# fdrmrc/Polydeal

Hardware: AMD Instinct MI355X
Metric: assembled DoF/s (SIP Poisson, p=3, 3D) (higher is better)
Workload: dtype f64

## Files before the change

polydeal_amd/csrc/pdh_capi.cpp:

```cpp
#include "pdh_basis.h"
#include "pdh_combos.h"
#include "pdh_ctx.h"
#include "pdh_kernels.h"
#include "pdh_moment_tables.h"

#include <hip/hip_runtime.h>

#include <algorithm>
#include <chrono>
#include <cmath>
#include <cstdio>
#include <cstdlib>
#include <cstring>
#include <memory>
#include <string>
#include <vector>

static pdh_resolve_fn g_resolve[PDH_N_GROUPS] = {pdh_resolve_g0, pdh_resolve_g1, pdh_resolve_g2, pdh_resolve_g3,
                                                 pdh_resolve_g4, pdh_resolve_g5, pdh_resolve_g6, pdh_resolve_g7};

template <int NT, int LB>
static constexpr int sched_instr(bool sym)
{
  int c = 0;
// ... 80 lines not shown
    (void)hipHostFree(ctx->pinned);
  for (auto &ev : ctx->events)
    if (ev)
      (void)hipEventDestroy(ev);
  (void)hipStreamDestroy(ctx->own_stream);
  if (ctx->stream2)
    (void)hipStreamDestroy(ctx->stream2);
  if (ctx->ev_fork)
    (void)hipEventDestroy(ctx->ev_fork);
  if (ctx->ev_join)
    (void)hipEventDestroy(ctx->ev_join);
  delete ctx;
}

extern "C" int pdh_terms_merge_stats(pdh_ctx *ctx, int64_t *out4)
{
  if (!ctx || !out4)
    return fail(ctx, PDH_EINVAL, "ctx and out4 are required");
  if (!ctx->prob.resident)
    return fail(ctx, PDH_ESTATE, "pdh_terms_merge_stats called before pdh_set_problem");
  for (int i = 0; i < 4; ++i)
    out4[i] = ctx->prob.row_kernel == RowKernel::terms ? ctx->prob.terms_merge[i] : 0;
  return PDH_OK;
}

struct GaussRule01
{
  double x[PDH_MAX_N1D] = {0}, w[PDH_MAX_N1D] = {0};
  explicit GaussRule01(int n)
  {
    std::vector<long double> gx, gw;
    pdh::gauss_legendre01(n, gx, gw);
    for (int i = 0; i < n; ++i)
      x[i] = (double)gx[i], w[i] = (double)gw[i];
  }
};

static int pack_faces_on_device(pdh_ctx *ctx, const pdh_problem *p, const Packed &K, PdhDev &D)
{
  const int dim = p->dim;
  const int64_t nap = K.n_ap, nqf = K.nqf_src, nruns = (int64_t)K.pk_at.size();
  double *out[5] = {nullptr, nullptr, nullptr, nullptr, nullptr};
  const size_t out_n[5] = {(size_t)dim * nap, (size_t)dim * nap, (size_t)nap, (size_t)nap, (size_t)nap};
  for (int k = 0; k < 5; ++k)
    PDH_TRY(device_buffer(ctx, out_n[k], &out[k], "packed face points"));
  D.ap_x = out[0], D.ap_n = out[1], D.ap_wself = out[2], D.ap_wcross = out[3], D.ap_sig = out[4];
  if (nruns == 0 || nap == 0)
    return PDH_OK;
  Staging st(ctx);
  const double *d_x = nullptr, *d_n = nullptr, *d_w = nullptr, *d_wo = nullptr;
  if (K.cart)
    {
      const pdh_cartesian_points *cp = K.cart;
      const int64_t nsf = nqf / ((int64_t)cp->nqf * cp->nqf);
      const double *d_box = nullptr;
      const int32_t *d_cell = nullptr, *d_face = nullptr;
      double *x = nullptr, *n = nullptr, *w = nullptr;
      PDH_TRY(st.upload(cp->cell_box, (size_t)cp->n_cells * 6, &d_box, "cell boxes"));
      PDH_TRY(st.upload(cp->fq_cell, (size_t)nsf, &d_cell, "cells of the sub-faces"));
      PDH_TRY(st.upload(cp->fq_face, (size_t)nsf, &d_face, "local faces of the sub-faces"));
      PDH_TRY(st.alloc((size_t)dim * nqf, &x, "face points"));
      PDH_TRY(st.alloc((size_t)dim * nqf, &n, "face normals"));
      PDH_TRY(st.alloc((size_t)nqf, &w, "face weights"));
      const GaussRule01 g(cp->nqf);
      PDH_HIP(ctx, pdh_launch_gen_faces(cp->nqf, g.x, g.w, d_box, d_cell, d_face, nqf, x, n, w, ctx->stream));
      d_x = x, d_n = n, d_w = w;
    }
  else
    {
      PDH_TRY(st.upload(p->fq_x, (size_t)dim * nqf, &d_x, "face points"));
      PDH_TRY(st.upload(p->fq_n, (size_t)dim * nqf, &d_n, "face normals"));
      PDH_TRY(st.upload(p->fq_w, (size_t)nqf, &d_w, "face weights"));
      if (p->fq_w_out)
        PDH_TRY(st.upload(p->fq_w_out, (size_t)nqf, &d_wo, "face weights of side 1"));
    }
  const int64_t *d_at = nullptr, *d_fq = nullptr;
  const int32_t *d_cnt = nullptr, *d_fl = nullptr;
  const double *d_sg = nullptr;
  PDH_TRY(st.upload(K.pk_at.data(), K.pk_at.size(), &d_at, "face runs: packed position"));
  PDH_TRY(st.upload(K.pk_fq.data(), K.pk_fq.size(), &d_fq, "face runs: caller position"));
  PDH_TRY(st.upload(K.pk_cnt.data(), K.pk_cnt.size(), &d_cnt, "face runs: counts"));
  PDH_TRY(st.upload(K.pk_flags.data(), K.pk_flags.size(), &d_fl, "face runs: flags"));
  PDH_TRY(st.upload(K.pk_sig.data(), K.pk_sig.size(), &d_sg, "face runs: sigma"));
  PDH_HIP(ctx, pdh_launch_pack_faces(dim, nqf, d_x, d_n, d_w, d_wo, nruns, d_at, d_fq, d_cnt, d_fl, d_sg, nap, out[0], out[1], out[2],
                                     out[3], out[4], ctx->stream));
  PDH_HIP(ctx, hipStreamSynchronize(ctx->stream));
  return PDH_OK;
}

static int generate_volume_points(pdh_ctx *ctx, const Packed &K, PdhDev &D)
{
  const pdh_cartesian_points *cart = K.cart;
  const int64_t m3 = (int64_t)cart->nq * cart->nq * cart->nq, ngroups = K.n_vq / m3;
  std::vector<int32_t> gcell((size_t)std::max<int64_t>(ngroups, 1));
  for (int sl = 0; sl < K.n_owned; ++sl)
    {
      const int64_t g0 = K.vq_ptr[sl] / m3, g1 = K.vq_ptr[sl + 1] / m3, src = K.vq_src[sl] / m3;
      for (int64_t g = g0; g < g1; ++g)
        gcell[(size_t)g] = cart->vq_cell[src + (g - g0)];
    }
  double *x = nullptr, *w = nullptr;
  PDH_TRY(device_buffer(ctx, (size_t)3 * K.n_vq, &x, "volume points"));
  PDH_TRY(device_buffer(ctx, (size_t)K.n_vq, &w, "volume weights"));
  Staging st(ctx);
  const double *d_box = nullptr;
  const int32_t *d_gcell = nullptr;
  PDH_TRY(st.upload(cart->cell_box, (size_t)cart->n_cells * 6, &d_box, "cell boxes"));
  PDH_TRY(st.upload(gcell.data(), gcell.size(), &d_gcell, "cells of the volume rules"));
  const GaussRule01 g(cart->nq);
  PDH_HIP(ctx, pdh_launch_gen_volume(cart->nq, g.x, g.w, d_box, d_gcell, K.n_vq, x, K.n_vq, w, ctx->stream));
  PDH_HIP(ctx, hipStreamSynchronize(ctx->stream));
  D.vq_x = x, D.vq_w = w;
  return PDH_OK;
}

static int upload_problem(pdh_ctx *ctx, const pdh_problem *p, const Packed &K)
{
  PdhDev &D = ctx->prob.dev;
  std::memset(&D, 0, sizeof(D));
  D.dim = p->dim;
  D.n = K.n;
  D.n1d = K.n1d;
  D.diag_first = p->diag_first ? 1 : 0;
  D.reaction_c = p->reaction_c;
  D.tab = K.tab;
  D.vq_stride = K.vq_stride_h;
  D.ap_stride = K.n_ap;
  const std::vector<double> bbox(p->bbox, p->bbox + (size_t)p->n_agg * 2 * p->dim);
  PDH_UP(bbox, D.bbox);
  PDH_UP(K.midx, D.midx);
  PDH_UP(K.vq_ptr, D.vq_ptr);
  if (K.cart)
    PDH_TRY(generate_volume_points(ctx, K, D));
  else
    {
      PDH_TRY(upload(ctx, K.vqx_h, (size_t)p->dim * K.vq_stride_h, &D.vq_x, "D.vq_x"));
      PDH_TRY(upload(ctx, K.vqw_h, (size_t)K.n_vq, &D.vq_w, "D.vq_w"));
    }
  PDH_UP(K.ap_ptr, D.ap_ptr);
  PDH_TRY(pack_faces_on_device(ctx, p, K, D));
  PDH_UP(K.own_agg, D.own_agg);
  PDH_UP(K.own_row, D.own_row);
  PDH_UP(K.row_base, D.row_base);
  PDH_UP(K.row_len, D.row_len);
  PDH_UP(K.diag_L, D.diag_L);
  PDH_UP(K.it_own, D.it_own);
  PDH_UP(K.it_nbr, D.it_nbr);
  PDH_UP(K.it_pbeg, D.it_pbeg);
  PDH_UP(K.it_pcnt, D.it_pcnt);
  PDH_UP(K.it_pos, D.it_pos);
  PDH_UP(K.it_nbr_slot, D.it_nbr_slot);
  PDH_UP(K.it_pos_t, D.it_pos_t);
  PDH_TRY(upload(ctx, K.blk_ptr, &ctx->prob.d_blk_ptr, "ctx->d_blk_ptr"));
  PDH_TRY(upload(ctx, K.blk_dof, &ctx->prob.d_blk_dof, "ctx->d_blk_dof"));
  if (K.ghost)
    {
      PDH_TRY(upload(ctx, K.r21_src, &ctx->prob.d_r21_src, "ctx->d_r21_src"));
      PDH_TRY(upload(ctx, K.r21_dst, &ctx->prob.d_r21_dst, "ctx->d_r21_dst"));
      PDH_TRY(upload(ctx, K.r21_rlen, &ctx->prob.d_r21_rlen, "ctx->d_r21_rlen"));
      PDH_TRY(upload(ctx, K.r22_ptr, &ctx->prob.d_r22_ptr, "ctx->d_r22_ptr"));
      PDH_TRY(upload(ctx, K.r22_src, &ctx->prob.d_r22_src, "ctx->d_r22_src"));
      PDH_TRY(upload(ctx, K.r22_slot, &ctx->prob.d_r22_slot, "ctx->d_r22_slot"));
    }
  PDH_TRY(device_buffer(ctx, (size_t)(K.n_values + K.n_send), &D.values, "values"));
  PDH_TRY(upload(ctx, K.vq_src, &ctx->prob.d_vq_src, "ctx->d_vq_src"));
  if (p->dim == 3 && K.n1d >= 2 && K.n1d <= 4)
    {
      const std::vector<double> mt = pdh::moment_tables(p->degree, p->basis);
      if ((int)mt.size() != pdhm::moment_table_doubles(K.n1d))
        return fail(ctx, PDH_EDEVICE, "moment tables: the host's and the kernels' sizes differ");
      PDH_TRY(upload(ctx, mt, &ctx->prob.d_mtab, "ctx->d_mtab"));
    }
  return PDH_OK;
}

static void record_problem(pdh_ctx *ctx, const pdh_problem *p, const Packed &K)
{
  ctx->prob.ghost = K.ghost;
  ctx->prob.n_send = K.n_send;
  ctx->prob.n_recv = K.n_recv;
  ctx->prob.send_count = K.send_count;
  ctx->prob.recv_count = K.recv_count;
  ctx->prob.n_r21 = (int)K.r21_src.size();
  ctx->prob.n_r22 = (int)K.r22_slot.size();
  ctx->prob.n_values = K.n_values;
  ctx->prob.n_owned = K.n_owned;
  ctx->prob.n_diag_slots = (int)K.own_agg.size();
  ctx->prob.n_items = (int)K.it_own.size();
  ctx->prob.n_vq = K.n_vq;
  ctx->prob.n_ap = K.n_ap;
  ctx->prob.NT = K.NT;
  ctx->prob.tiled = K.tiled;
  ctx->prob.basis = p->basis;
  ctx->prob.n_vq_caller = p->vq_ptr[p->n_agg];
  ctx->prob.n_fq_caller = p->n_faces ? p->fq_ptr[p->n_faces] : 0;
  ctx->prob.cart_fq_face.clear();
  ctx->prob.cart_nqf = 0;
  if (K.cart && K.cart->nqf > 0)
    {
      ctx->prob.cart_nqf = K.cart->nqf;
      ctx->prob.cart_fq_face.assign(K.cart->fq_face, K.cart->fq_face + ctx->prob.n_fq_caller / ((int64_t)K.cart->nqf * K.cart->nqf));
    }
  ctx->prob.face_runs.clear();
  ctx->prob.face_runs.reserve(K.run_ap.size());
  for (size_t r = 0; r < K.run_ap.size(); ++r)
    ctx->prob.face_runs.push_back({K.run_ap[r], K.run_fq[r], K.run_cnt[r], K.run_bdry[r], K.run_slot[r]});
  ctx->prob.n_rows_owned = (int64_t)K.n_owned * K.n;
  ctx->prob.n_rows_total = p->n_rows;
  ctx->prob.max_row_len = K.max_row_len;
  ctx->prob.h_blk_ptr = K.blk_ptr;
  ctx->prob.h_blk_dof = K.blk_dof;
  ctx->prob.h_slot_dof.resize((size_t)K.n_owned);
  for (int s = 0; s < K.n_owned; ++s)
    ctx->prob.h_slot_dof[(size_t)s] = p->dof_offset[K.own_agg[(size_t)s]];
  ctx->prob.n_agg_total = p->n_agg;
  const int64_t i_sym = sched_instr_rt(K.NT, K.LB, true), i_full = sched_instr_rt(K.NT, K.LB, false);
  const int ch_d = (K.NT >= 3) ? 64 : 32, ch_o = 32;
  auto ksteps = [](int64_t npts, int ch) {
    int64_t s = (npts / ch) * (ch / 4);
    const int64_t rem = npts % ch;
    return s + (rem + 3) / 4;
  };
  int64_t kv = 0, kf = 0, ko = 0;
  for (size_t sl = 0; sl < K.own_agg.size(); ++sl)
    {
      kv += ksteps(K.vq_ptr[sl + 1] - K.vq_ptr[sl], ch_d);
      kf += ksteps(K.ap_ptr[sl + 1] - K.ap_ptr[sl], ch_d);
    }
  for (size_t it = 0; it < K.it_pcnt.size(); ++it)
    ko += ksteps(K.it_pcnt[it], ch_o);
  ctx->prob.mfma_diag = kv * (p->dim + (p->reaction_c != 0.0 ? 1 : 0)) * i_sym + kf * 2 * i_sym;
  ctx->prob.mfma_offdiag = ko * 2 * i_full;
  if (K.tiled)
    {
      const int64_t nt = (K.n + 63) / 64, i64 = sched_instr_rt(4, 4, true);
      ctx->prob.mfma_diag = (kv * (p->dim + (p->reaction_c != 0.0 ? 1 : 0)) + kf * 2) * (64 * (nt * (nt - 1) / 2) + i64 * nt);
      ctx->prob.mfma_offdiag = ko * 2 * 64 * nt * nt;
    }
}

static int upload_rows_state(pdh_ctx *ctx, const Packed &K, const KernelPlan &plan, int cus)
{
  const RowsHost &RH = plan.rows;
  PdhRows &R = ctx->prob.rows;
  PDH_UP(RH.fr_ptr, R.fr_ptr);
  PDH_UP(RH.fr_pbeg, R.fr_pbeg);
  PDH_UP(RH.fr_pcnt, R.fr_pcnt);
  PDH_UP(RH.fr_nbr, R.fr_nbr);
  PDH_UP(RH.fr_axis, R.fr_axis);
  PDH_UP(RH.fr_blk, R.fr_blk);
  PDH_UP(RH.fr_flags, R.fr_flags);
  PDH_UP(RH.fr_coord, R.fr_coord);
  PDH_UP(RH.fr_sigma, R.fr_sigma);
  PDH_UP(RH.fr_nsign, R.fr_nsign);
  PDH_UP(RH.meta, R.meta);
  PDH_TRY(device_buffer(ctx, 16, &R.sched, "row kernel: work counter"));
  PDH_HIP(ctx, hipMemset(R.sched, 0, 16 * sizeof(unsigned int)));
  const size_t n_stamps = (size_t)std::max(K.n_owned, 1) * 16;
  PDH_TRY(device_buffer(ctx, n_stamps, &R.stamps, "row kernel: stamps"));
  PDH_HIP(ctx, hipMemset(R.stamps, 0, n_stamps * sizeof(long long)));
  if (RH.multi)
    {
      const int waves = cus * 8;
      const size_t stride = std::max<size_t>((size_t)RH.maxf * 64, (size_t)RH.maxs * 32 + 64);
      PDH_TRY(device_buffer(ctx, (size_t)waves * stride, &R.m2c_scratch, "row kernel: MULTI scratch"));
      R.scratch_waves = waves;
      R.scratch_stride = (int64_t)stride;
    }
  R.tensor_only = plan.tensor_only ? 1 : 0;
  R.multi = RH.multi ? 1 : 0;
  R.maxe = RH.maxe;
  R.maxf = RH.maxf;
  R.vq_tensor_n = plan.vq_n;
  R.fq_tensor_n = RH.fq_tensor_n;
  return PDH_OK;
}

static int upload_terms_state(pdh_ctx *ctx, const Packed &K, const KernelPlan &plan)
{
  const TermsHost &TH = plan.terms;
  PdhTerms &T = ctx->prob.terms;
  PDH_UP(TH.meta, T.meta);
  PDH_UP(TH.sf_pt, T.sf_pt);
  PDH_UP(TH.sf_info, T.sf_info);
  PDH_UP(TH.sf_ivl, T.sf_ivl);
  PDH_UP(TH.cell_ivl, T.cell_ivl);
  T.maxruns = TH.maxruns, T.maxsf = TH.maxsf, T.maxsi = TH.maxsi, T.maxcell = TH.maxcell;
  T.vq_tensor_n = plan.vq_n, T.fq_tensor_n = plan.rows.fq_tensor_n;
  T.lds_bytes = TH.lds_bytes;
  T.split = TH.split;
  T.task_pts = TH.task_pts;
  T.tpm = TH.task_pts > 4 ? 8 : 4;
  T.tstride = pdht::terms_task_doubles(T.maxsf, T.maxcell, T.tpm);
  const size_t n_tdata = (size_t)std::max(K.n_owned, 1) * T.tstride;
  double *tdata = nullptr;
  PDH_TRY(device_buffer(ctx, n_tdata, &tdata, "term kernel: records of 1-D rules"));
  PDH_HIP(ctx, hipMemsetAsync(tdata, 0, n_tdata * sizeof(double), ctx->stream));
  T.tdata = tdata;
  PDH_HIP(ctx, pdh_launch_terms_gather(&ctx->prob.dev, &T, tdata, K.n_owned, ctx->stream));
  PDH_HIP(ctx, hipStreamSynchronize(ctx->stream));
  const size_t n_stamps = (size_t)std::max(K.n_owned, 1) * 16;
  PDH_TRY(device_buffer(ctx, n_stamps, &T.stamps, "term kernel: stamps"));
  PDH_HIP(ctx, hipMemset(T.stamps, 0, n_stamps * sizeof(long long)));
  ctx->prob.terms_merge[0] = TH.n_cells_in, ctx->prob.terms_merge[1] = TH.n_cells_out;
  ctx->prob.terms_merge[2] = TH.n_sf_in, ctx->prob.terms_merge[3] = TH.n_sf_out;
  return PDH_OK;
}

static void resolve_launches(pdh_ctx *ctx, const Packed &K, const PlanSwitches &sw, int cus)
{
  pdh_ctx::Problem &pr = ctx->prob;
  const PdhDev &D = pr.dev;
  const bool reaction = D.reaction_c != 0.0;
  if (K.tiled)
    pdh_resolve_tiled(D.dim, D.n1d, D.n, reaction, pr.n_diag_slots, pr.n_items, pr.direct);
  else
    g_resolve[combo_group(D.dim, D.n1d, K.NT, K.LB)](D.dim, D.n1d, K.NT, K.LB, reaction, pr.n_diag_slots, pr.n_items, pr.direct);
  if (pr.d_mtab)
    pdh_resolve_moment(D.n1d, D.n, pr.n_diag_slots, pr.n_items, pr.moment);
  if (pr.row_kernel == RowKernel::rows)
    pr.row = pdh_resolve_rows(&D, &pr.rows, pr.n_owned, cus, sw.rows_waves_per_cu, sw.rows_lds_pad, sw.rows_verbose, &pr.row_zero_sched);
  else if (pr.row_kernel == RowKernel::terms)
    pr.row = pdh_resolve_terms(&D, &pr.terms, pr.n_owned, sw.terms_wg_waves);
}

static int set_problem_impl(pdh_ctx *ctx, const pdh_problem *p, int32_t row_begin, int32_t row_end, const pdh_cartesian_points *cart);

extern "C" int pdh_set_problem_local(pdh_ctx *ctx, const pdh_problem *p, int32_t row_begin, int32_t row_end)
{
  return set_problem_impl(ctx, p, row_begin, row_end, nullptr);
}

extern "C" int pdh_set_problem_cartesian(pdh_ctx *ctx, const pdh_problem *p, const pdh_cartesian_points *points, int32_t row_begin,
                                         int32_t row_end)
{
  if (!points)
    return fail(ctx, PDH_EINVAL, "points is NULL");
  return set_problem_impl(ctx, p, row_begin, row_end, points);
}

static int set_problem_impl(pdh_ctx *ctx, const pdh_problem *p, int32_t row_begin, int32_t row_end, const pdh_cartesian_points *cart)
{
  PDH_TRY(need_ctx(ctx));
  if (cart && ctx->exchange_mode == PDH_EXCHANGE_GHOST)
    return fail(ctx, PDH_EUNSUPPORTED, "the cartesian description runs owner-computes-rows only (no ghost-block exchange)");
  PDH_HIP(ctx, hipSetDevice(ctx->device));
  PDH_HIP(ctx, hipStreamSynchronize(ctx->stream));
  free_problem(ctx);
  ++ctx->values_gen;
  ++ctx->problem_epoch;
  struct FreeUnlessDone
  {
    pdh_ctx *ctx;
    bool done = false;
    ~FreeUnlessDone()
    {
      if (!done)
        free_problem(ctx);
    }
  } guard{ctx};
  const PlanSwitches sw = read_plan_switches();
  auto t_last = std::chrono::steady_clock::now();
  auto lap = [&](const char *what) {
    if (!sw.trace)
      return;
    const auto now = std::chrono::steady_clock::now();
    fprintf(stderr, "[pdh_set_problem] %-32s %7.1f ms\n", what, std::chrono::duration<double, std::milli>(now - t_last).count());
    t_last = now;
  };
  lap("wait for the stream, free the old problem");

  std::unique_ptr<Packed> K_owner(new Packed);
  Packed &K = *K_owner;
  PDH_TRY(pack_problem(ctx->err, p, row_begin, row_end, K, ctx->exchange_mode, cart));
  lap("validate + repack (host)");
  auto plan = std::make_unique<KernelPlan>(plan_kernels(p, K, sw));
  lap("row kernel plan (host)");
  if (cart && plan->kernel != RowKernel::terms)
    return fail(ctx, PDH_EUNSUPPORTED, "cartesian description: the term kernels do not apply (a polytope's tables exceed their LDS budget, "
                                       "or the element has none): describe the problem with its points (pdh_set_problem)");
  PDH_TRY(upload_problem(ctx, p, K));
  record_problem(ctx, p, K);
  lap("upload: state of every kernel");
  int cus = 256;
  (void)hipDeviceGetAttribute(&cus, hipDeviceAttributeMultiprocessorCount, ctx->device);
  if (plan->kernel == RowKernel::rows)
    {
      PDH_TRY(upload_rows_state(ctx, K, *plan, cus));
      lap("upload: pdh_rows.h state");
    }
  else if (plan->kernel == RowKernel::terms)
    {
      PDH_TRY(upload_terms_state(ctx, K, *plan));
      lap("upload: term kernel state");
    }
  ctx->prob.row_kernel = plan->kernel;
  ctx->prob.why_terms = plan->why_terms;
  resolve_launches(ctx, K, sw, cus);
  ctx->prob.resident = true;
  ctx->ev_used = 0;
  guard.done = true;
  K_owner.reset();
  plan.reset();
  lap("release host staging");
  return PDH_OK;
}

extern "C" int pdh_set_algorithm(pdh_ctx *ctx, int algorithm)
{
  PDH_TRY(need_ctx(ctx));
  if (algorithm != PDH_ALG_AUTO && algorithm != PDH_ALG_DIRECT && algorithm != PDH_ALG_MOMENT && algorithm != PDH_ALG_ROWS)
    return fail(ctx, PDH_EINVAL, "algorithm must be PDH_ALG_AUTO, PDH_ALG_DIRECT, PDH_ALG_MOMENT or PDH_ALG_ROWS");
  ctx->algorithm = algorithm;
  return PDH_OK;
}

extern "C" int pdh_algorithm_in_use(pdh_ctx *ctx)
{
  if (!resident(ctx))
    return fail(ctx, PDH_ESTATE, "no problem resident");
  if (ctx->use_rows())
    return PDH_ALG_ROWS;
  const bool d = ctx->use_moment(0), o = ctx->use_moment(1);
  return d && o ? PDH_ALG_MOMENT : (d || o ? PDH_ALG_MIXED : PDH_ALG_DIRECT);
}

extern "C" int pdh_rows_kernel_in_use(pdh_ctx *ctx)
{
  if (!resident(ctx))
    return fail(ctx, PDH_ESTATE, "no problem resident");
  if (!ctx->use_rows())
    return PDH_ROWS_NONE;
  if (ctx->prob.row_kernel == RowKernel::terms)
    return PDH_ROWS_TERMS;
  if (ctx->prob.rows.multi)
    return PDH_ROWS_MULTI;
  return ctx->prob.dev.n == 64 ? PDH_ROWS_PIECES : PDH_ROWS_STREAMED;
}

extern "C" int pdh_set_problem(pdh_ctx *ctx, const pdh_problem *p)
{
  if (!p)
    return fail(ctx, PDH_EINVAL, "problem is NULL");
  return pdh_set_problem_local(ctx, p, 0, p->n_rows);
}

static int take_events(pdh_ctx *ctx, hipEvent_t (&e)[4])
{
  for (hipEvent_t &x : e)
    x = ctx->next_event();
  if (!e[0] || !e[1] || !e[2] || !e[3])
    return fail(ctx, PDH_EDEVICE, "hipEventCreate failed");
  return PDH_OK;
}

extern "C" int pdh_assemble_device(pdh_ctx *ctx)
{
  PDH_TRY(need_problem(ctx, "pdh_assemble_device"));
  ++ctx->values_gen;
  PDH_HIP(ctx, hipSetDevice(ctx->device));
  pdh_ctx::Problem &pr = ctx->prob;
  if (ctx->algorithm == PDH_ALG_MOMENT && !ctx->prob.d_mtab)
    return fail(ctx, PDH_EUNSUPPORTED, "the moment form exists for 3-D bases of degree 1..3 only");
  if (ctx->algorithm == PDH_ALG_ROWS && ctx->prob.row_kernel == RowKernel::none)
    return fail(ctx, PDH_EUNSUPPORTED, "the row kernel does not apply to the resident problem (3-D FE_DGQ / FE_AggloDGP of degree 1 .. 3 on polytopes whose faces are unions of axis-aligned planes, no exchange variant; pdh_check_rows says why)");
  pr.has_values = true;
  pr.galerkin_values = false;
  if (ctx->use_rows())
    {
      hipEvent_t ev[4] = {nullptr, nullptr, nullptr, nullptr};
      if (ctx->profiling)
        {
          PDH_TRY(take_events(ctx, ev));
          PDH_HIP(ctx, hipEventRecord(ev[0], ctx->stream));
        }
      if (pr.row_kernel == RowKernel::terms)
        PDH_HIP(ctx, pdh_launch_terms(&pr.row, &pr.dev, &pr.terms, pr.n_owned, ctx->stream));
      else
        PDH_HIP(ctx, pdh_launch_rows(&pr.row, pr.row_zero_sched, &pr.dev, &pr.rows, pr.d_mtab, pr.n_owned, ctx->stream));
      if (ctx->profiling)
        {
          PDH_HIP(ctx, hipEventRecord(ev[1], ctx->stream));
          PDH_HIP(ctx, hipEventRecord(ev[2], ctx->stream));
          PDH_HIP(ctx, hipEventRecord(ev[3], ctx->stream));
        }
      return PDH_OK;
    }
  hipEvent_t ev[4] = {nullptr, nullptr, nullptr, nullptr};
  if (ctx->profiling)
    PDH_TRY(take_events(ctx, ev));
  hipEvent_t e0 = ev[0], e1 = ev[1], f0 = ev[2], f1 = ev[3];
  const bool ov = ctx->overlapped();
  hipStream_t sd = ctx->stream, so = ov ? ctx->stream2 : ctx->stream;
  const bool graphable = !ctx->profiling && !ov && ctx->prob.n_values < pdh_ctx::small_values;
  if (graphable && ctx->prob.graph_state == 1 && (ctx->prob.graph_alg != ctx->algorithm || ctx->prob.graph_stream != ctx->stream))
    ctx->prob.drop_graph();
  if (graphable && ctx->prob.graph_state == 1)
    {
      PDH_HIP(ctx, hipGraphLaunch(ctx->prob.graph_exec, ctx->stream));
      return PDH_OK;
    }
  bool capturing = false;
  if (graphable && ctx->prob.graph_state == 0)
    {
      if (hipStreamBeginCapture(ctx->stream, hipStreamCaptureModeThreadLocal) == hipSuccess)
        capturing = true;
      else
        {
          (void)hipGetLastError();
          ctx->prob.graph_state = -1;
        }
    }
  auto end_capture = [&](bool ok) {
    if (!capturing)
      return;
    hipGraph_t g = nullptr;
    hipError_t e = hipStreamEndCapture(ctx->stream, &g);
    if (ok && e == hipSuccess && g && hipGraphInstantiate(&ctx->prob.graph_exec, g, nullptr, nullptr, 0) == hipSuccess)
      {
        ctx->prob.graph_state = 1;
        ctx->prob.graph_alg = ctx->algorithm;
        ctx->prob.graph_stream = ctx->stream;
      }
    else
      {
        (void)hipGetLastError();
        ctx->prob.graph_exec = nullptr;
        ctx->prob.graph_state = -1;
      }
    if (g)
      (void)hipGraphDestroy(g);
  };
  auto launch_blocks = [&](int k, int count, hipStream_t s) {
    if (ctx->use_moment(k))
      return pdh_launch_moment(&pr.moment[k], &pr.dev, pr.d_mtab, count, s);
    if (!pr.tiled)
      return pdh_launch_direct(&pr.direct[k], &pr.dev, count, s);
    const hipError_t e = pdh_launch_tiled(&pr.direct[k], &pr.dev, count, s);
    return k == 0 && e == hipSuccess ? pdh_launch_tiled(&pr.direct[2], &pr.dev, count, s) : e;
  };
  if (ov)
    {
      PDH_HIP(ctx, hipEventRecord(ctx->ev_fork, ctx->stream));
      PDH_HIP(ctx, hipStreamWaitEvent(ctx->stream2, ctx->ev_fork, 0));
    }
  if (ctx->profiling)
    PDH_HIP(ctx, hipEventRecord(e0, sd));
  {
    const hipError_t le = launch_blocks(0, pr.n_diag_slots, sd);
    if (le != hipSuccess)
      {
        end_capture(false);
        return fail(ctx, PDH_EDEVICE, std::string("diagonal-block kernel: ") + hipGetErrorString(le));
      }
  }
  if (ctx->profiling)
    PDH_HIP(ctx, hipEventRecord(e1, sd));
  if (ctx->profiling)
    PDH_HIP(ctx, hipEventRecord(f0, so));
  {
    const hipError_t le = launch_blocks(1, pr.n_items, so);
    if (le != hipSuccess)
      {
        end_capture(false);
        return fail(ctx, PDH_EDEVICE, std::string("coupling-block kernel: ") + hipGetErrorString(le));
      }
  }
  if (ctx->profiling)
    PDH_HIP(ctx, hipEventRecord(f1, so));
  if (ov)
    {
      PDH_HIP(ctx, hipEventRecord(ctx->ev_join, ctx->stream2));
      PDH_HIP(ctx, hipStreamWaitEvent(ctx->stream, ctx->ev_join, 0));
    }
  if (capturing)
    {
      end_capture(true);
      if (ctx->prob.graph_state == 1)
        PDH_HIP(ctx, hipGraphLaunch(ctx->prob.graph_exec, ctx->stream));
      else
        return pdh_assemble_device(ctx);
    }
  return PDH_OK;
}

extern "C" int pdh_set_exchange_mode(pdh_ctx *ctx, int mode)
{
  PDH_TRY(need_ctx(ctx));
  if (mode != PDH_EXCHANGE_NONE && mode != PDH_EXCHANGE_GHOST)
    return fail(ctx, PDH_EINVAL, "mode must be PDH_EXCHANGE_NONE or PDH_EXCHANGE_GHOST");
  ctx->exchange_mode = mode;
  return PDH_OK;
}

extern "C" int pdh_exchange_layout(pdh_ctx *ctx, int n_ranks, int64_t *send_count, int64_t *recv_count)
{
  if (!resident(ctx))
    return fail(ctx, PDH_ESTATE, "no problem resident");
  if (!ctx->prob.ghost)
    return fail(ctx, PDH_ESTATE, "the resident problem was not set in PDH_EXCHANGE_GHOST mode");
  if (n_ranks < (int)ctx->prob.send_count.size() || !send_count || !recv_count)
    return fail(ctx, PDH_EINVAL, "n_ranks is smaller than the number of ranks in agg_rank, or an output is NULL");
  for (int r = 0; r < n_ranks; ++r)
    {
      send_count[r] = r < (int)ctx->prob.send_count.size() ? ctx->prob.send_count[r] : 0;
      recv_count[r] = r < (int)ctx->prob.recv_count.size() ? ctx->prob.recv_count[r] : 0;
    }
  return PDH_OK;
}

extern "C" int pdh_exchange_get_send(pdh_ctx *ctx, double *d_send)
{
  if (!resident(ctx) || !ctx->prob.ghost)
    return fail(ctx, PDH_ESTATE, "no problem resident in PDH_EXCHANGE_GHOST mode");
  if (ctx->prob.n_send == 0)
    return PDH_OK;
  if (!d_send)
    return fail(ctx, PDH_EINVAL, "d_send is NULL");
  PDH_HIP(ctx, hipSetDevice(ctx->device));
  PDH_HIP(ctx, hipMemcpyAsync(d_send, ctx->prob.dev.values + ctx->prob.n_values, ctx->prob.n_send * sizeof(double), hipMemcpyDeviceToDevice,
                              ctx->stream));
  return PDH_OK;
}

extern "C" int pdh_exchange_apply(pdh_ctx *ctx, const double *d_recv)
{
  if (!resident(ctx) || !ctx->prob.ghost)
    return fail(ctx, PDH_ESTATE, "no problem resident in PDH_EXCHANGE_GHOST mode");
  ++ctx->values_gen;
  if (ctx->prob.n_recv == 0)
    return PDH_OK;
  if (!d_recv)
    return fail(ctx, PDH_EINVAL, "d_recv is NULL");
  PDH_HIP(ctx, hipSetDevice(ctx->device));
  PDH_HIP(ctx, pdh_launch_ghost_apply(&ctx->prob.dev, d_recv, ctx->prob.n_r21, ctx->prob.d_r21_src, ctx->prob.d_r21_dst, ctx->prob.d_r21_rlen, ctx->prob.n_r22,
                                      ctx->prob.d_r22_ptr, ctx->prob.d_r22_src, ctx->prob.d_r22_slot, ctx->stream));
  return PDH_OK;
}

extern "C" int pdh_set_stream(pdh_ctx *ctx, void *stream)
{
  PDH_TRY(need_ctx(ctx));
  PDH_HIP(ctx, hipSetDevice(ctx->device));
  PDH_HIP(ctx, hipStreamSynchronize(ctx->stream));
  ctx->stream = stream ? (hipStream_t)stream : ctx->own_stream;
  return PDH_OK;
}

extern "C" int pdh_debug_rows_stamps(pdh_ctx *ctx, long long *out)
{
  const long long *src = !ctx || !ctx->prob.resident ? nullptr
                         : ctx->prob.row_kernel == RowKernel::terms ? ctx->prob.terms.stamps
                         : ctx->prob.row_kernel == RowKernel::rows ? ctx->prob.rows.stamps
                                                                : nullptr;
  if (!src || !out)
    return fail(ctx, PDH_ESTATE, "no row-kernel problem resident");
  PDH_HIP(ctx, hipSetDevice(ctx->device));
  PDH_HIP(ctx, hipStreamSynchronize(ctx->stream));
  PDH_HIP(ctx, hipMemcpy(out, src, (size_t)ctx->prob.n_owned * 16 * sizeof(long long), hipMemcpyDeviceToHost));
  return PDH_OK;
}

extern "C" int pdh_set_overlap(pdh_ctx *ctx, int enabled)
{
  PDH_TRY(need_ctx(ctx));
  ctx->overlap = enabled != 0;
  return PDH_OK;
}

extern "C" int pdh_synchronize(pdh_ctx *ctx)
{
  PDH_TRY(need_ctx(ctx));
  PDH_HIP(ctx, hipSetDevice(ctx->device));
  PDH_HIP(ctx, hipStreamSynchronize(ctx->stream));
  return PDH_OK;
}

extern "C" void *pdh_stream(pdh_ctx *ctx) { return ctx ? (void *)ctx->stream : nullptr; }

extern "C" int pdh_assemble(pdh_ctx *ctx, double *values)
{
  if (!values)
    return fail(ctx, PDH_EINVAL, "values is NULL");
  int rc = pdh_assemble_device(ctx);
  if (rc != PDH_OK)
    return rc;
  PDH_HIP(ctx, hipMemcpyAsync(values, ctx->prob.dev.values, ctx->prob.n_values * sizeof(double), hipMemcpyDeviceToHost, ctx->stream));
  PDH_HIP(ctx, hipStreamSynchronize(ctx->stream));
  return PDH_OK;
}

extern "C" int pdh_copy_values(pdh_ctx *ctx, double *values)
{
  if (!resident(ctx))
    return fail(ctx, PDH_ESTATE, "no problem resident");
  if (!values)
    return fail(ctx, PDH_EINVAL, "values is NULL");
  PDH_HIP(ctx, hipSetDevice(ctx->device));
  PDH_HIP(ctx, hipMemcpyAsync(values, ctx->prob.dev.values, ctx->prob.n_values * sizeof(double), hipMemcpyDeviceToHost, ctx->stream));
  PDH_HIP(ctx, hipStreamSynchronize(ctx->stream));
  return PDH_OK;
}

extern "C" int pdh_values_checksum(pdh_ctx *ctx, double *out4)
{
  if (!resident(ctx))
    return fail(ctx, PDH_ESTATE, "no problem resident");
  if (!out4)
    return fail(ctx, PDH_EINVAL, "out4 is NULL");
  PDH_HIP(ctx, hipSetDevice(ctx->device));
  double *d = ctx->checksum.get<double>(4);
  if (!d)
    return fail(ctx, PDH_EDEVICE, "pdh_values_checksum: out of device memory");
  hipError_t e = pdh_launch_checksum(ctx->prob.dev.values, ctx->prob.n_values, d, ctx->stream);
  if (e == hipSuccess)
    e = hipMemcpyAsync(out4, d, 4 * sizeof(double), hipMemcpyDeviceToHost, ctx->stream);
  if (e == hipSuccess)
    e = hipStreamSynchronize(ctx->stream);
  if (e != hipSuccess)
    return fail(ctx, PDH_EDEVICE, std::string("pdh_values_checksum: ") + hipGetErrorString(e));
  return PDH_OK;
}

extern "C" int pdh_assemble_sip_local(pdh_ctx *ctx, const pdh_problem *p, int32_t row_begin, int32_t row_end, double *values)
{
  int rc = pdh_set_problem_local(ctx, p, row_begin, row_end);
  if (rc != PDH_OK)
    return rc;
  return pdh_assemble(ctx, values);
}

extern "C" int pdh_assemble_sip(pdh_ctx *ctx, const pdh_problem *p, double *values)
{
  if (!p)
    return fail(ctx, PDH_EINVAL, "problem is NULL");
  return pdh_assemble_sip_local(ctx, p, 0, p->n_rows, values);
}
extern "C" int pdh_device_values(pdh_ctx *ctx, double **device_ptr, int64_t *n_values)
{
  if (!resident(ctx))
    return fail(ctx, PDH_ESTATE, "no problem resident");
  if (device_ptr)
    *device_ptr = ctx->prob.dev.values;
  if (n_values)
    *n_values = ctx->prob.n_values;
  return PDH_OK;
}

extern "C" int pdh_set_profiling(pdh_ctx *ctx, int enabled)
{
  PDH_TRY(need_ctx(ctx));
  PDH_HIP(ctx, hipSetDevice(ctx->device));
  PDH_HIP(ctx, hipStreamSynchronize(ctx->stream));
  ctx->profiling = enabled != 0;
  ctx->ev_used = 0;
  return PDH_OK;
}

extern "C" int pdh_kernel_times_ms(pdh_ctx *ctx, float *ms, int *n_launches)
{
  if (!ctx || !ms)
    return fail(ctx, PDH_EINVAL, "ctx or ms is NULL");
  const size_t nl = ctx->ev_used / 4;
  if (nl == 0)
    return fail(ctx, PDH_ESTATE, "no profiled launch recorded (pdh_set_profiling(1) then pdh_assemble_device)");
  PDH_HIP(ctx, hipSetDevice(ctx->device));
  PDH_HIP(ctx, hipStreamSynchronize(ctx->stream));
  double sum[PDH_N_KERNELS] = {0.0, 0.0};
  for (size_t l = 0; l < nl; ++l)
    for (int k = 0; k < PDH_N_KERNELS; ++k)
      {
        float t = 0.f;
        PDH_HIP(ctx, hipEventElapsedTime(&t, ctx->events[4 * l + 2 * k], ctx->events[4 * l + 2 * k + 1]));
        sum[k] += t;
      }
  for (int k = 0; k < PDH_N_KERNELS; ++k)
    ms[k] = (float)(sum[k] / (double)nl);
  if (n_launches)
    *n_launches = (int)nl;
  return PDH_OK;
}

extern "C" int pdh_kernel_work(pdh_ctx *ctx, int64_t *mfma_instr)
{
  if (!resident(ctx) || !mfma_instr)
    return fail(ctx, PDH_ESTATE, "no problem resident");
  mfma_instr[0] = (ctx->use_moment(0) || ctx->use_rows()) ? 0 : ctx->prob.mfma_diag;
  mfma_instr[1] = (ctx->use_moment(1) || ctx->use_rows()) ? 0 : ctx->prob.mfma_offdiag;
  return PDH_OK;
}

extern "C" int pdh_problem_stats(pdh_ctx *ctx, int64_t *stats)
{
  if (!resident(ctx) || !stats)
    return fail(ctx, PDH_ESTATE, "no problem resident");
  stats[0] = ctx->prob.n_owned;
  stats[1] = ctx->prob.n_items;
  stats[2] = ctx->prob.n_vq;
  stats[3] = ctx->prob.n_ap;
  stats[4] = ctx->prob.n_values;
  stats[5] = ctx->prob.dev.n;
  stats[6] = (int64_t)pdh::lds_bytes_diag(ctx->prob.dev.dim, ctx->prob.dev.n1d, ctx->prob.NT);
  stats[7] = (int64_t)pdh::lds_bytes_offdiag(ctx->prob.dev.dim, ctx->prob.dev.n1d, ctx->prob.NT);
  return PDH_OK;
}
```

polydeal_amd/csrc/pdh_exchange.hip:

```cpp
#include "pdh_kernels.h"
#include "pdh_launch.h"

__global__ void __launch_bounds__(PDH_WAVE) k_ghost_apply(const PdhDev P, const double *__restrict__ recv, const int n_r21,
                                                          const int64_t *__restrict__ r21_src, const int64_t *__restrict__ r21_dst,
                                                          const int32_t *__restrict__ r21_rlen, const int n_r22,
                                                          const int64_t *__restrict__ r22_ptr, const int64_t *__restrict__ r22_src,
                                                          const int32_t *__restrict__ r22_slot)
{
  const int lane = threadIdx.x, item = blockIdx.x, n = P.n;
  if (lane >= n)
    return;
  if (item < n_r21)
    {
      const double *src = recv + r21_src[item] + lane;
      double *dst = P.values + r21_dst[item] + lane;
      const int64_t rlen = r21_rlen[item];
      for (int R = 0; R < n; ++R)
        dst[R * rlen] = src[(int64_t)R * n];
    }
  else if (item < n_r21 + n_r22)
    {
      const int k = item - n_r21, slot = r22_slot[k];
      const int64_t rlen = P.row_len[slot];
      const int dest = (P.diag_first && lane == 0) ? 0 : P.diag_L[slot] + lane;
      double *dst = P.values + P.row_base[slot] + dest;
      const int64_t sb = r22_ptr[k], se = r22_ptr[k + 1];
      for (int R = 0; R < n; ++R)
        {
          double acc = dst[R * rlen];
          for (int64_t s = sb; s < se; ++s)
            acc += recv[r22_src[s] + (int64_t)R * n + lane];
          dst[R * rlen] = acc;
        }
    }
}

extern "C" hipError_t pdh_launch_ghost_apply(const PdhDev *P, const double *recv, int n_r21, const int64_t *r21_src,
                                             const int64_t *r21_dst, const int32_t *r21_rlen, int n_r22, const int64_t *r22_ptr,
                                             const int64_t *r22_src, const int32_t *r22_slot, hipStream_t stream)
{
  const int count = n_r21 + n_r22;
  if (count <= 0)
    return hipSuccess;
  hipLaunchKernelGGL(k_ghost_apply, dim3((unsigned)count), dim3(PDH_WAVE), 0, stream, *P, recv, n_r21, r21_src, r21_dst, r21_rlen,
                     n_r22, r22_ptr, r22_src, r22_slot);
  return hipGetLastError();
}

__global__ void __launch_bounds__(256) k_checksum(const double *__restrict__ v, const int64_t n, double *__restrict__ out)
{
  double s = 0.0, sa = 0.0, mx = 0.0, bad = 0.0;
  for (int64_t i = (int64_t)blockIdx.x * blockDim.x + threadIdx.x; i < n; i += (int64_t)gridDim.x * blockDim.x)
    {
      const double x = v[i];
      if (isfinite(x))
        {
          s += x;
          sa += fabs(x);
          mx = fmax(mx, fabs(x));
        }
      else
        bad += 1.0;
    }
  for (int o = 32; o > 0; o >>= 1)
    {
      s += __shfl_down(s, o);
      sa += __shfl_down(sa, o);
      bad += __shfl_down(bad, o);
      mx = fmax(mx, __shfl_down(mx, o));
    }
  if ((threadIdx.x & 63) == 0)
    {
      atomicAdd(out + 0, s);
      atomicAdd(out + 1, sa);
      atomicAdd(out + 3, bad);
      atomicMax(reinterpret_cast<unsigned long long *>(out + 2), (unsigned long long)__double_as_longlong(mx));
    }
}

extern "C" hipError_t pdh_launch_checksum(const double *values, int64_t n, double *d_out4, hipStream_t stream)
{
  hipError_t e = hipMemsetAsync(d_out4, 0, 4 * sizeof(double), stream);
  if (e != hipSuccess || n <= 0)
    return e;
  hipLaunchKernelGGL(k_checksum, dim3(2048), dim3(256), 0, stream, values, n, d_out4);
  return hipGetLastError();
}

__global__ void __launch_bounds__(256) k_pack_faces(const int dim, const int64_t nqf, const double *__restrict__ fq_x,
                                                    const double *__restrict__ fq_n, const double *__restrict__ fq_w,
                                                    const double *__restrict__ fq_w_out, const int64_t n_runs,
                                                    const int64_t *__restrict__ pk_at, const int64_t *__restrict__ pk_fq,
                                                    const int32_t *__restrict__ pk_cnt, const int32_t *__restrict__ pk_flags,
                                                    const double *__restrict__ pk_sig, const int64_t nap, double *__restrict__ ap_x,
                                                    double *__restrict__ ap_n, double *__restrict__ ap_wself,
                                                    double *__restrict__ ap_wcross, double *__restrict__ ap_sig)
{
  const int lane = threadIdx.x & (PDH_WAVE - 1);
  const int64_t r = (int64_t)blockIdx.x * (blockDim.x / PDH_WAVE) + (threadIdx.x / PDH_WAVE);
  if (r >= n_runs)
    return;
  const int64_t at = pk_at[r], fq = pk_fq[r];
  const int cnt = pk_cnt[r], fl = pk_flags[r];
  const bool side0 = (fl & 1) != 0, bdry = (fl & 2) != 0;
  const double sig = pk_sig[r], sgn = side0 ? 1.0 : -1.0;
  for (int t = lane; t < cnt; t += PDH_WAVE)
    {
      const int64_t q = fq + t, a = at + t;
      const double w_in = fq_w[q], w_out = fq_w_out ? fq_w_out[q] : w_in;
      ap_wself[a] = bdry ? 2.0 * w_in : (side0 ? w_in : w_out);
      ap_wcross[a] = bdry ? 0.0 : w_out;
      ap_sig[a] = sig;
      for (int c = 0; c < dim; ++c)
        {
          ap_x[c * nap + a] = fq_x[c * nqf + q];
          ap_n[c * nap + a] = sgn * fq_n[c * nqf + q];
        }
    }
}

extern "C" hipError_t pdh_launch_pack_faces(int dim, int64_t nqf, const double *fq_x, const double *fq_n, const double *fq_w,
                                            const double *fq_w_out, int64_t n_runs, const int64_t *pk_at, const int64_t *pk_fq,
                                            const int32_t *pk_cnt, const int32_t *pk_flags, const double *pk_sig, int64_t nap,
                                            double *ap_x, double *ap_n, double *ap_wself, double *ap_wcross, double *ap_sig,
                                            hipStream_t stream)
{
  if (n_runs <= 0)
    return hipSuccess;
  const int per_block = 256 / PDH_WAVE;
  const int64_t blocks = (n_runs + per_block - 1) / per_block;
  hipLaunchKernelGGL(k_pack_faces, dim3((unsigned)blocks), dim3(256), 0, stream, dim, nqf, fq_x, fq_n, fq_w, fq_w_out, n_runs, pk_at,
                     pk_fq, pk_cnt, pk_flags, pk_sig, nap, ap_x, ap_n, ap_wself, ap_wcross, ap_sig);
  return hipGetLastError();
}
```

polydeal_amd/csrc/pdh_launch.h:

```cpp
#pragma once
#include <hip/hip_runtime.h>
#include <stdint.h>

#include <type_traits>

#include "pdh_dev.h"
#include "pdh_rows_tables.h"
#include "pdh_solve.h"
#include "pdh_terms_tables.h"

struct PdhTransferArgs;
struct PdhGalerkinArgs;

struct PdhLaunch
{
  const void *kernel;
  unsigned grid, block;
  size_t lds;
};

typedef void (*PdhDirectKernel)(PdhDev, int);
typedef void (*PdhTiledKernel)(PdhDev, int, int);
typedef void (*PdhMomentKernel)(PdhDev, const double *, int);
typedef void (*PdhRowsKernel)(PdhDev, PdhRows, const double *, int);
typedef void (*PdhTermsKernel)(PdhDev, PdhTerms, int);

template <class... A>
inline PdhLaunch pdh_record(void (*kernel)(A...), long long grid, unsigned block, size_t lds)
{
  return grid > 0x7fffffffLL ? PdhLaunch{} : PdhLaunch{(const void *)kernel, (unsigned)(grid > 0 ? grid : 0), block, lds};
}
template <class... A>
inline hipError_t pdh_launch_as(void (*)(A...), const PdhLaunch &L, hipStream_t stream, A... a)
{
  if (!L.kernel)
    return hipErrorInvalidValue;
  if (!L.grid)
    return hipSuccess;
  void *args[] = {&a...};
  (void)hipLaunchKernel(L.kernel, dim3(L.grid), dim3(L.block), args, L.lds, stream);
  return hipGetLastError();
}
template <class F>
inline void pdh_for_bools(F &&f)
{
  f();
}
template <class F, class... B>
inline void pdh_for_bools(F &&f, bool b, B... rest)
{
  if (b)
    pdh_for_bools([&](auto... c) { f(std::true_type{}, c...); }, rest...);
  else
    pdh_for_bools([&](auto... c) { f(std::false_type{}, c...); }, rest...);
}

extern "C" {
typedef void (*pdh_resolve_fn)(int dim, int n1d, int nt, int lb, bool reaction, int n_own, int n_items, PdhLaunch *L);
#define PDH_DECL(g) void pdh_resolve_g##g(int, int, int, int, bool, int, int, PdhLaunch *);
PDH_DECL(0) PDH_DECL(1) PDH_DECL(2) PDH_DECL(3) PDH_DECL(4) PDH_DECL(5) PDH_DECL(6) PDH_DECL(7)
#undef PDH_DECL
hipError_t pdh_launch_direct(const PdhLaunch *L, const PdhDev *P, int count, hipStream_t stream);

hipError_t pdh_launch_rhs(int dim, int n1d, const PdhDev *P, int count, const double *f_vol, const double *g_face, double *rhs,
                          const int64_t *vq_src, const int64_t *ap_src, const int64_t *bd_rng, hipStream_t stream);

hipError_t pdh_launch_eval(int dim, int n1d, int grad, const PdhDev *P, int count, const double *coef, const int64_t *pt_ptr,
                           const double *pts, int64_t pts_stride, double *out_u, double *out_g, int by_agg, hipStream_t stream);
hipError_t pdh_launch_shape(int dim, int n1d, const PdhDev *P, int n_boxes, const int64_t *pt_ptr, const double *pts,
                            int64_t pts_stride, double *out, hipStream_t stream);
hipError_t pdh_launch_eval_err(int dim, int n1d, const PdhDev *P, int count, const double *coef, const int64_t *pt_ptr,
                               const double *pts, int64_t pts_stride, const double *w, const double *exact_u, const double *exact_g,
                               double *err, hipStream_t stream);

void pdh_resolve_moment(int n1d, int n, int n_own, int n_items, PdhLaunch *L);
hipError_t pdh_launch_moment(const PdhLaunch *L, const PdhDev *P, const double *mtab, int count, hipStream_t stream);
PdhLaunch pdh_resolve_rows(const PdhDev *P, const PdhRows *R, int count, int cus, int waves_per_cu, size_t lds_pad, bool verbose,
                           bool *zero_sched);
hipError_t pdh_launch_rows(const PdhLaunch *L, bool zero_sched, const PdhDev *P, const PdhRows *R, const double *mtab, int count,
                           hipStream_t stream);

PdhLaunch pdh_resolve_terms(const PdhDev *P, const PdhTerms *T, int count, int wg_waves);
hipError_t pdh_launch_terms(const PdhLaunch *L, const PdhDev *P, const PdhTerms *T, int count, hipStream_t stream);
hipError_t pdh_launch_terms_gather(const PdhDev *P, const PdhTerms *T, double *out, int count, hipStream_t stream);

hipError_t pdh_launch_mf_tables(const PdhDev *P, const PdhTerms *T, double *tables, int count, hipStream_t stream);
hipError_t pdh_launch_mf_vmult(const PdhSolveArgs *A, int n1d, const PdhTerms *T, const double *tables, const double *x, double *y,
                               double *part, hipStream_t stream);

void pdh_resolve_tiled(int dim, int n1d, int n, bool reaction, int n_own, int n_items, PdhLaunch *L);
hipError_t pdh_launch_tiled(const PdhLaunch *L, const PdhDev *P, int count, hipStream_t stream);

hipError_t pdh_launch_gen_volume(int nq, const double *nodes, const double *weights, const double *d_box, const int32_t *d_gcell,
                                 int64_t n_points, double *vq_x, int64_t stride, double *vq_w, hipStream_t stream);
hipError_t pdh_launch_gen_faces(int nqf, const double *nodes, const double *weights, const double *d_box, const int32_t *d_cell,
                                const int32_t *d_face, int64_t n_points, double *fq_x, double *fq_n, double *fq_w, hipStream_t stream);

hipError_t pdh_launch_pack_faces(int dim, int64_t nqf, const double *fq_x, const double *fq_n, const double *fq_w,
                                 const double *fq_w_out, int64_t n_runs, const int64_t *pk_at, const int64_t *pk_fq,
                                 const int32_t *pk_cnt, const int32_t *pk_flags, const double *pk_sig, int64_t nap, double *ap_x,
                                 double *ap_n, double *ap_wself, double *ap_wcross, double *ap_sig, hipStream_t stream);
hipError_t pdh_launch_ghost_apply(const PdhDev *P, const double *recv, int n_r21, const int64_t *r21_src, const int64_t *r21_dst,
                                  const int32_t *r21_rlen, int n_r22, const int64_t *r22_ptr, const int64_t *r22_src,
                                  const int32_t *r22_slot, hipStream_t stream);
hipError_t pdh_launch_checksum(const double *values, int64_t n, double *d_out4, hipStream_t stream);

hipError_t pdh_launch_vmult(const PdhSolveArgs *A, const double *x, double *y, double *part, hipStream_t stream);
hipError_t pdh_launch_block_inverse(const PdhSolveArgs *A, double *dinv, int32_t *flag, hipStream_t stream);
hipError_t pdh_launch_diag_inverse(const PdhSolveArgs *A, double *dinv, int32_t *flag, hipStream_t stream);
hipError_t pdh_launch_cg_update(const PdhSolveArgs *A, int mode, int kind, const double *dinv, const double *b, const double *q,
                                const double *p, double *x, double *r, double *z, const double *scal, double *part, hipStream_t stream);
hipError_t pdh_launch_cheb_update(const PdhSolveArgs *A, int first, int kind, const double *dinv, const double *b, const double *q,
                                  double *d, double *r, double *x, double c1, double c2, int zero_start, const double *rcg, double *part,
                                  hipStream_t stream);
hipError_t pdh_launch_cg_direction(int64_t n_rows, int init, const double *z, double *p, const double *scal, hipStream_t stream);
hipError_t pdh_launch_cg_finalise(const double *part, int n_owned, int stage, double *scal, hipStream_t stream);

hipError_t pdh_launch_dense_gather(const PdhSolveArgs *A, double *D, int ld, int n_rows, hipStream_t stream);
hipError_t pdh_launch_dense_cholesky(double *U, int ld, int n_rows, double *dg, double *piv, int32_t *flag, hipStream_t stream);
hipError_t pdh_launch_dense_inverse(const double *U, const double *dg, int ld, int n_rows, double *Wd, double *G, hipStream_t stream);
hipError_t pdh_launch_dense_symv(const PdhSolveArgs *A, const double *G, int ld, int n_rows, const double *r, double *z,
                                 const double *rcg, double *part, hipStream_t stream);

hipError_t pdh_launch_prolongate(int dim, int n1d, int add, const PdhTransferArgs *A, const double *coarse, double *fine, hipStream_t stream);
hipError_t pdh_launch_restrict(int dim, int n1d, int add, const PdhTransferArgs *A, const double *fine, double *coarse, hipStream_t stream);
hipError_t pdh_launch_residual_sub(int64_t n_rows, const double *b, double *r, hipStream_t stream);

hipError_t pdh_launch_galerkin(int dim, int n1d, const PdhGalerkinArgs *A, hipStream_t stream);
}
```

polydeal_amd/csrc/pdh_plan.cpp:

```cpp
#include "pdh_plan_internal.h"

#include "pdh_basis.h"
#include "pdh_combos.h"
#include "pdh_rows_tables.h"
#include "pdh_terms_tables.h"

#include <chrono>
#include <cstdio>

static thread_local std::string g_err_noctx;
std::string &pdh_noctx_error() { return g_err_noctx; }

int combo_group(int dim, int n1d, int nt, int lb)
{
#define PDH_X(G, D, N, T, L)                                                                       \
  if (dim == D && n1d == N && nt == T && lb == L)                                                  \
    return G;
  PDH_COMBOS(PDH_X)
#undef PDH_X
  return -1;
}


namespace
// ... 1091 lines not shown
  static thread_local std::vector<TermsSfGeom> gs;
  gs.resize((size_t)ns);
  for (int g = 0; g < ns; ++g)
    {
      S.sf_geom(t, g, gs[(size_t)g]);
      gs[(size_t)g].fj = RH.fast_j[3 * t + gs[(size_t)g].c] == 1 ? 1 : 0;
    }
  auto single = [&](int g) {
    TermsMerged::Sf f{};
    f.pb = K.run_ap[t] + g * gsz;
    f.c = gs[(size_t)g].c, f.pos = gs[(size_t)g].pos, f.fj = gs[(size_t)g].fj, f.ni = f.nj = 1;
    out.push_back(f);
  };
  if (mf <= 1 || ns <= 1)
    {
      for (int g = 0; g < ns; ++g)
        single(g);
      return;
    }
  static thread_local std::vector<char> used, ftaken;
  static thread_local std::vector<int> mem, ii, jj, fgrid;
  static thread_local std::vector<double> ki, kj;
  used.assign((size_t)ns, 0);
  for (int g0 = 0; g0 < ns; ++g0)
    {
      if (used[(size_t)g0])
        continue;
      const TermsSfGeom r0 = gs[(size_t)g0];
      mem.clear();
      for (int g = g0; g < ns; ++g)
        if (!used[(size_t)g] && gs[(size_t)g].c == r0.c && gs[(size_t)g].pos == r0.pos && gs[(size_t)g].fj == r0.fj &&
            std::fabs(gs[(size_t)g].z - r0.z) <= 1e-9 * S.hbox[r0.c])
          {
            mem.push_back(g);
            used[(size_t)g] = 1;
          }
      const int c = r0.c, ti = c == 0 ? 1 : 0, tj = c == 2 ? 1 : 2;
      int nd[3] = {0, 0, 1};
      bool ok = mem.size() > 1;
      if (ok)
        {
          ki.resize(mem.size()), kj.resize(mem.size());
          for (size_t m = 0; m < mem.size(); ++m)
            ki[m] = gs[(size_t)mem[m]].xi, kj[m] = gs[(size_t)mem[m]].xj;
          nd[0] = cluster_1d(ki, 1e-9 * S.hbox[ti], ii), nd[1] = cluster_1d(kj, 1e-9 * S.hbox[tj], jj);
          ok = (int64_t)nd[0] * nd[1] <= 4096;
        }
      if (ok)
        {
          fgrid.assign((size_t)nd[0] * nd[1], -1);
          for (size_t m = 0; m < mem.size() && ok; ++m)
            {
              int &gg = fgrid[(size_t)(ii[m] + nd[0] * jj[m])];
              ok = gg < 0;
              gg = (int)m;
            }
        }
      if (!ok)
        {
          for (int g : mem)
            single(g);
          continue;
        }
      auto atm = [&](int i, int j, int = 0) { return fgrid[(size_t)(i + nd[0] * j)]; };
      auto at = [&](int i, int j) { return mem[(size_t)atm(i, j)]; };
      const int mx[3] = {mf, mf, 1};
      ftaken.assign(mem.size(), 0);
      cover_grid(
        nd, mx, ftaken, atm,
        [&](int m, const int *o) {
          return S.sf_fits(t, mem[(size_t)m], at(ii[(size_t)m], o[1]), at(o[0], jj[(size_t)m]), at(o[0], o[1]), ti, tj, r0.fj);
        },
        [&](const int *o, const int *best) {
          TermsMerged::Sf f;
          const int go = at(o[0], o[1]);
          f.pb = K.run_ap[t] + go * gsz;
          f.c = c, f.pos = r0.pos, f.fj = r0.fj;
          f.ni = best[0], f.nj = best[1];
          for (int q = 0; q < TERMS_MI; ++q)
            {
              f.ivl[0][q] = q < best[0] ? (int32_t)((at(o[0] + q, o[1]) - go) * gsz) : 0;
              f.ivl[1][q] = q < best[1] ? (int32_t)((at(o[0], o[1] + q) - go) * gsz) : 0;
            }
          out.push_back(f);
        });
    }
}

template <class Src>
void merge_terms_of_slot(const Src &S, const RowsHost &RH, const std::vector<size_t> &order, bool enabled, TermsMerged &M)
{
  const Packed &K = S.K;
  const int tn = S.tn, fn = S.fn;
  const int ncell = (int)((K.vq_ptr[S.sl + 1] - K.vq_ptr[S.sl]) / S.m3);
  const int mc = tn >= 1 && tn <= 4 ? std::min(TERMS_MI, 8 / tn) : 1;
  if (!(enabled && mc > 1 && ncell > 1 && merge_cells(S, ncell, mc, M.cells)))
    {
      M.cells.resize((size_t)ncell);
      for (int u = 0; u < ncell; ++u)
        for (int d = 0; d < 3; ++d)
          for (int i = 0; i < TERMS_MI; ++i)
            M.cells[(size_t)u].ivl[d][i] = i == 0 ? u : -1;
    }
  const int mf = enabled && fn >= 1 && fn <= 4 ? std::min(TERMS_MI, 8 / fn) : 1;
  M.run_off.assign(order.size() + 1, 0);
  size_t tot = 0;
  for (size_t t : order)
    tot += (size_t)(K.run_cnt[t] / S.gsz);
  M.sfs.reserve(tot);
  M.n_in = ncell + (int64_t)tot;
  for (size_t e = 0; e < order.size(); ++e)
    {
      merge_sub_faces(S, order[e], RH, mf, M.sfs);
      M.run_off[e + 1] = (int)M.sfs.size();
      M.nsf += (int)M.run_size(e);
      if (K.run_nbr[order[e]] >= 0)
        M.nsi += (int)M.run_size(e);
    }
  for (const auto &f : M.sfs)
    M.ivl_f = std::max(M.ivl_f, std::max(f.ni, f.nj));
  for (const auto &c : M.cells)
    for (int d = 0; d < 3; ++d)
      {
        int k = 0;
        for (int i = 0; i < TERMS_MI; ++i)
          k += c.ivl[d][i] >= 0 ? 1 : 0;
        M.ivl_c = std::max(M.ivl_c, k);
      }
}

void merge_terms(const pdh_problem *p, const Packed &K, const RowsHost &RH, const FaceAnalysis &A, int tn, bool enabled,
                 std::vector<TermsMerged> &MG)
{
  MG.assign((size_t)K.n_owned, TermsMerged());
  host_parallel_for((size_t)K.n_owned, [&](size_t sl) {
    if (K.cart)
      merge_terms_of_slot(FromBoxes(p, K, sl, tn, RH.fq_tensor_n), RH, A.order[sl], enabled, MG[sl]);
    else
      merge_terms_of_slot(FromPoints(p, K, sl, tn, RH.fq_tensor_n), RH, A.order[sl], enabled, MG[sl]);
  });
}

constexpr int PDH_TERMS_LDS_CAP = 40 * 1024;

bool check_runs_of_slots(const Packed &K, const FaceAnalysis &A, int64_t gsz, int64_t m3, TermsHost &T, std::string *why)
{
  for (int sl = 0; sl < K.n_owned; ++sl)
    {
      const auto &idx = A.order[(size_t)sl];
      int nb = 0;
      for (size_t t : idx)
        {
          if (K.run_cnt[t] % gsz)
            return refuse(why, "term kernel: a face is not made of whole sub-face rules");
          if (K.run_nbr[t] < 0)
            ++nb;
        }
      if (nb > 1)
        return refuse(why, "term kernel: more than one boundary run on a polytope");
      const int64_t nq = K.vq_ptr[sl + 1] - K.vq_ptr[sl];
      if (nq % m3 || nq / m3 > 65535 || idx.size() > 250)
        return refuse(why, "term kernel: too many cells or faces on a polytope");
      T.maxruns = std::max<int>(T.maxruns, (int)idx.size());
    }
  if (A.n_ordered != K.run_ap.size())
    return refuse(why, "run bookkeeping");
  T.maxruns = std::max(T.maxruns, 1);
  return true;
}

bool write_terms_of_slot(const pdh_problem *p, const Packed &K, const std::vector<size_t> &idx, const TermsMerged &M, size_t sl, TermsHost &T)
{
  constexpr int HDR = pdht::TERMS_HDR, ENT = pdht::TERMS_ENT;
  double *rec = T.meta.data() + sl * (HDR + T.maxruns * ENT);
  const int64_t at0 = (int64_t)sl * T.maxsf;
  int64_t at = at0;
  int nsfb = 0, e = 0;
  bool ok = true;
  for (size_t t : idx)
    {
      const TermsMerged::Sf *fs = M.run_begin((size_t)e);
      const int ns = (int)M.run_size((size_t)e);
      double *en = rec + HDR + e * ENT;
      en[0] = as_d((long long)(uint32_t)(at - at0) | ((long long)ns << 32));
      en[1] = as_d((long long)K.run_blk[t]);
      en[2] = K.run_sig[t];
      write_box(en + 3, en + 6, p, K.run_nbr[t]);
      if (K.run_nbr[t] < 0)
        {
          nsfb += ns;
          ok = ok && e == 0;
        }
      for (int q = 0; q < ns; ++q, ++at)
        {
          const TermsMerged::Sf &f = fs[q];
          T.sf_pt[(size_t)at] = f.pb;
          T.sf_info[(size_t)at] = e | (f.c << 8) | (f.pos << 10) | (f.fj << 11) | (f.ni << 12) | (f.nj << 15);
          for (int d = 0; d < 2; ++d)
            for (int i = 0; i < TERMS_MI; ++i)
              T.sf_ivl[((size_t)at * 2 + d) * TERMS_MI + i] = f.ivl[d][i];
        }
      ++e;
    }
  for (size_t u = 0; u < M.cells.size(); ++u)
    for (int d = 0; d < 3; ++d)
      for (int i = 0; i < TERMS_MI; ++i)
        T.cell_ivl[((sl * T.maxcell + u) * 3 + d) * TERMS_MI + i] = M.cells[u].ivl[d][i];
  rec[0] = as_d((long long)idx.size() | ((long long)M.cells.size() << 16) | ((long long)nsfb << 32));
  write_slot_header(rec, p, K, sl);
  rec[10] = as_d(K.vq_ptr[sl]), rec[11] = as_d((long long)(at - at0));
  return ok;
}
}

bool build_terms_tables(const pdh_problem *p, const Packed &K, const RowsHost &RH, const FaceAnalysis &A, int vq_n, const PlanSwitches &sw,
                        TermsHost &T, std::string *why)
{
  const int basis = p->basis == PDH_BASIS_AGGLODGP ? 1 : 0;
  if (p->dim != 3 || !pdht::terms_has_kind(K.n1d, basis))
    return refuse(why, "term kernel: 3-D FE_DGQ(1,2) / FE_AggloDGP(1..3) only");
  if (!RH.planar_ok)
    return refuse(why, "term kernel: needs faces that are unions of axis-aligned planes");
  if (RH.fq_tensor_n <= 0)
    return refuse(why, "term kernel: needs tensor-product rules on every sub-face (the face points are not, to the rounding bound of the geometry)");
  if (vq_n <= 0)
    return refuse(why, "term kernel: needs tensor-product rules on every sub-cell (the volume points are not, to the rounding bound of the geometry)");
  if ((int)K.own_agg.size() != K.n_owned)
    return refuse(why, "term kernel: exchange variant");
  const int fn = RH.fq_tensor_n;
  const int64_t m3 = (int64_t)vq_n * vq_n * vq_n;
  if (!check_runs_of_slots(K, A, (int64_t)fn * fn, m3, T, why))
    return false;
  auto tnow = [] { return std::chrono::steady_clock::now(); };
  auto t_prev = tnow();
  auto tlap = [&](const char *what) {
    if (sw.trace)
      fprintf(stderr, "[build_terms_tables] %-28s %6.1f ms\n", what, std::chrono::duration<double, std::milli>(tnow() - t_prev).count());
    t_prev = tnow();
  };
  tlap("run order");
  std::vector<TermsMerged> MG;
  merge_terms(p, K, RH, A, vq_n, sw.terms_merge != 0, MG);
  if (sw.terms_merge == 1)
    {
      int64_t n_in = 0, n_out = 0;
      for (const auto &m : MG)
        n_in += m.n_in, n_out += (int64_t)m.cells.size() + m.nsf;
      if (3 * n_out > 2 * n_in)
        merge_terms(p, K, RH, A, vq_n, false, MG);
    }
  tlap("merge");
  int ivl_c = 1, ivl_f = 1;
  for (int sl = 0; sl < K.n_owned; ++sl)
    {
      const TermsMerged &M = MG[(size_t)sl];
      ivl_c = std::max(ivl_c, M.ivl_c), ivl_f = std::max(ivl_f, M.ivl_f);
      T.n_sf_out += M.nsf;
      T.n_sf_in += M.n_in - (K.vq_ptr[sl + 1] - K.vq_ptr[sl]) / m3;
      T.n_cells_in += (K.vq_ptr[sl + 1] - K.vq_ptr[sl]) / m3;
      T.n_cells_out += (int64_t)M.cells.size();
      if (M.nsf > 65535)
        return refuse(why, "term kernel: too many sub-faces on a polytope");
      T.maxsf = std::max(T.maxsf, M.nsf);
      T.maxsi = std::max(T.maxsi, M.nsi);
      T.maxcell = std::max<int>(T.maxcell, (int)M.cells.size());
    }
  T.task_pts = std::max(vq_n * ivl_c, fn * ivl_f);
  tlap("maxima");
  {
    const int one = pdht::terms_lds_bytes(K.n1d, basis, T.maxruns, T.maxsf, T.maxsi, T.maxcell, 0);
    const int two = pdht::terms_lds_bytes(K.n1d, basis, T.maxruns, T.maxsf, T.maxsi, T.maxcell, 1);
    auto waves = [](int bytes) { return bytes <= 0 ? 0 : std::min(12, (int)(160 * 1024 / (((int64_t)bytes + 1279) / 1280 * 1280))); };
    T.split = sw.terms_split >= 0 ? sw.terms_split : ((waves(two) > waves(one) && K.n <= 20) ? 1 : 0);
    if (pdht::terms_has_kind(K.n1d, basis) == 2)
      T.split = 0;
    T.lds_bytes = T.split ? two : one;
  }
  if (T.lds_bytes <= 0 || T.lds_bytes > PDH_TERMS_LDS_CAP)
    return refuse(why, "term kernel: the tables of the largest polytope do not fit its LDS budget (moment-based kinds take over)");
  T.maxsf = std::max(T.maxsf, 1);
  T.maxcell = std::max(T.maxcell, 1);
  T.sf_pt.assign((size_t)K.n_owned * T.maxsf, 0);
  T.sf_info.assign((size_t)K.n_owned * T.maxsf, 0);
  T.sf_ivl.assign((size_t)K.n_owned * T.maxsf * 2 * TERMS_MI, 0);
  T.cell_ivl.assign((size_t)K.n_owned * T.maxcell * 3 * TERMS_MI, -1);
  T.meta.assign((size_t)K.n_owned * (pdht::TERMS_HDR + T.maxruns * pdht::TERMS_ENT), 0.0);
  const bool ok = host_parallel_all((size_t)K.n_owned, [&](size_t sl) { return write_terms_of_slot(p, K, A.order[sl], MG[sl], sl, T); });
  tlap("tables");
  return ok || refuse(why, "term kernel: run order");
}

PlanSwitches read_plan_switches()
{
  PlanSwitches s;
  auto first = [](const char *name) { return getenv(name) ? getenv(name)[0] : '\0'; };
  s.terms_merge = first("PDH_TERMS_MERGE") == '0' ? 0 : (first("PDH_TERMS_MERGE") == '2' ? 2 : 1);
  s.terms_split = getenv("PDH_TERMS_SPLIT") ? (first("PDH_TERMS_SPLIT") == '1' ? 1 : 0) : -1;
  s.trace = getenv("PDH_TRACE_SETUP") != nullptr;
  s.rows_verbose = getenv("PDH_ROWS_VERBOSE") != nullptr;
  s.terms_off = first("PDH_TERMS") == '0';
  s.terms_dgq3_off = first("PDH_TERMS_DGQ3") == '0';
  s.rows_waves_per_cu = getenv("PDH_ROWS_WAVES_PER_CU") ? atoi(getenv("PDH_ROWS_WAVES_PER_CU")) : 0;
  s.rows_lds_pad = getenv("PDH_ROWS_LDS_PAD") ? (size_t)atol(getenv("PDH_ROWS_LDS_PAD")) : 0;
  s.terms_wg_waves = getenv("PDH_TERMS_WG_WAVES") && atoi(getenv("PDH_TERMS_WG_WAVES")) == 8 ? 8 : 4;
  return s;
}

KernelPlan plan_kernels(const pdh_problem *p, const Packed &K, const PlanSwitches &sw)
{
  KernelPlan P;
  RowsHost &RH = P.rows;
  FaceAnalysis A;
  if (p->dim != 3 || K.n1d < 2 || K.n1d > 4 || K.ghost)
    {
      P.why_rows = P.why_terms = K.ghost ? "exchange variant" : "not 3-D FE_DGQ / FE_AggloDGP of degree 1 .. 3";
      return P;
    }
  if (K.cart)
    {
      RH.planar_ok = true;
      RH.fq_tensor_n = K.cart->nqf;
      RH.fast_j.assign(3 * K.run_ap.size(), 0);
      order_runs_of_slots(K, A);
      P.vq_n = K.cart->nq;
      P.why_rows = "cartesian description: the kinds of pdh_rows.h need the points";
    }
  else if (analyse_faces(p, K, RH, A, &P.why_rows) && build_rows_tables(p, K, A, sw, RH, &P.why_rows) &&
           rows_kind_applies(p, K, RH, P.vq_n, P.tensor_only, &P.why_rows))
    P.kernel = RowKernel::rows;
  const int terms_kind = pdht::terms_has_kind(K.n1d, p->basis == PDH_BASIS_AGGLODGP ? 1 : 0);
  if (!RH.planar_ok)
    P.why_terms = P.why_rows;
  else if (!K.cart && (sw.terms_off || (terms_kind == 2 && sw.terms_dgq3_off)))
    P.why_terms = "term kernel: switched off (PDH_TERMS / PDH_TERMS_DGQ3)";
  else
    {
      if (P.vq_n < 0 && RH.fq_tensor_n > 0)
        P.vq_n = resolve_volume_rules(p, K);
      if (build_terms_tables(p, K, RH, A, std::max(P.vq_n, 0), sw, P.terms, &P.why_terms))
        P.kernel = RowKernel::terms;
    }
  return P;
}

static int check_plan(const pdh_problem *p, int32_t row_begin, int32_t row_end, KernelPlan &plan)
{
  Packed K;
  g_err_noctx.clear();
  PDH_TRY(pack_problem(g_err_noctx, p, row_begin, row_end, K));
  PlanSwitches sw = read_plan_switches();
  sw.terms_off = sw.terms_dgq3_off = false;
  plan = plan_kernels(p, K, sw);
  return PDH_OK;
}

extern "C" int pdh_check_rows(const pdh_problem *p, int32_t row_begin, int32_t row_end)
{
  KernelPlan plan;
  PDH_TRY(check_plan(p, row_begin, row_end, plan));
  if (plan.kernel != RowKernel::none)
    return 1;
  g_err_noctx = plan.why_rows;
  if (plan.rows.planar_ok && plan.rows.fq_tensor_n > 0 && plan.vq_n > 0)
    g_err_noctx += "; " + plan.why_terms;
  return 0;
}

extern "C" int pdh_check_terms(const pdh_problem *p, int32_t row_begin, int32_t row_end, int64_t *stats5)
{
  KernelPlan plan;
  PDH_TRY(check_plan(p, row_begin, row_end, plan));
  const TermsHost &TH = plan.terms;
  if (stats5 && plan.rows.planar_ok)
    {
      stats5[0] = TH.maxruns, stats5[1] = TH.maxsf, stats5[2] = TH.maxsi, stats5[3] = TH.maxcell, stats5[4] = TH.lds_bytes;
    }
  if (plan.kernel == RowKernel::terms)
    return 1;
  g_err_noctx = plan.why_terms;
  return 0;
}

extern "C" int pdh_check_problem(const pdh_problem *p, int32_t row_begin, int32_t row_end, int64_t *stats)
{
  Packed K;
  g_err_noctx.clear();
  const int rc = pack_problem(g_err_noctx, p, row_begin, row_end, K);
  if (rc == PDH_OK && stats)
    {
      stats[0] = (int64_t)K.n_owned;
      stats[1] = (int64_t)K.it_own.size();
      stats[2] = K.n_vq;
      stats[3] = K.n_ap;
      stats[4] = K.n_values;
      stats[5] = K.n;
      stats[6] = (int64_t)pdh::lds_bytes_diag(p->dim, K.n1d, K.NT);
      stats[7] = (int64_t)pdh::lds_bytes_offdiag(p->dim, K.n1d, K.NT);
    }
  return rc;
}

extern "C" int pdh_check_exchange(const pdh_problem *p, int32_t row_begin, int32_t row_end, int n_ranks, int64_t *send_count,
                                  int64_t *recv_count)
{
  Packed K;
  g_err_noctx.clear();
  const int rc = pack_problem(g_err_noctx, p, row_begin, row_end, K, PDH_EXCHANGE_GHOST);
  if (rc != PDH_OK)
    return rc;
  if (n_ranks < (int)K.send_count.size() || !send_count || !recv_count)
    return fail(g_err_noctx, PDH_EINVAL, "n_ranks is smaller than the number of ranks in agg_rank, or an output is NULL");
  for (int r = 0; r < n_ranks; ++r)
    {
      send_count[r] = r < (int)K.send_count.size() ? K.send_count[r] : 0;
      recv_count[r] = r < (int)K.recv_count.size() ? K.recv_count[r] : 0;
    }
  return PDH_OK;
}

extern "C" int pdh_tridiagonal_eigenvalues(int k, const double *diag, const double *offdiag, double *lo, double *hi)
{
  g_err_noctx.clear();
  if (k < 1 || k > 256 || !diag || (k > 1 && !offdiag) || !lo || !hi)
    return fail(g_err_noctx, PDH_EINVAL, "pdh_tridiagonal_eigenvalues: 1 <= k <= 256, diag, offdiag (k > 1), lo and hi are required");
  double gl = diag[0], gu = diag[0], emax = 0.0;
  for (int i = 0; i < k; ++i)
    {
      const double el = i > 0 ? std::fabs(offdiag[i - 1]) : 0.0, er = i + 1 < k ? std::fabs(offdiag[i]) : 0.0;
      if (!std::isfinite(diag[i]) || !std::isfinite(el) || !std::isfinite(er))
        return fail(g_err_noctx, PDH_EINVAL, "pdh_tridiagonal_eigenvalues: entry " + std::to_string(i) + " is not finite");
      gl = std::min(gl, diag[i] - el - er);
      gu = std::max(gu, diag[i] + el + er);
      emax = std::max(emax, er);
    }
  if (k == 1)
    {
      *lo = *hi = diag[0];
      return PDH_OK;
    }
  const double norm = std::max(std::fabs(gl), std::fabs(gu));
  const double pivmin = std::max(2.2250738585072014e-308, 2.2250738585072014e-308 * emax * emax);
  const double pad = 2.0 * 2.220446049250313e-16 * norm * k + 2.0 * pivmin;
  gl -= pad;
  gu += pad;
  auto below = [&](double x) {
    int c = 0;
    double q = diag[0] - x;
    if (std::fabs(q) < pivmin)
      q = -pivmin;
    c += q < 0.0;
    for (int i = 1; i < k; ++i)
      {
        q = diag[i] - x - offdiag[i - 1] * offdiag[i - 1] / q;
        if (std::fabs(q) < pivmin)
          q = -pivmin;
        c += q < 0.0;
      }
    return c;
  };
  auto kth = [&](int want) {
    double a = gl, b = gu;
    for (int it = 0; it < 2200; ++it)
      {
        const double m = a + 0.5 * (b - a);
        if (!(m > a && m < b))
          break;
        if (below(m) <= want)
          a = m;
        else
          b = m;
      }
    return a + 0.5 * (b - a);
  };
  *lo = kth(0);
  *hi = kth(k - 1);
  return PDH_OK;
}

void pdh_lanczos_tridiagonal(const std::vector<double> &alpha, const std::vector<double> &beta, std::vector<double> &diag,
                             std::vector<double> &offdiag)
{
  const int m = (int)alpha.size();
  diag.assign((size_t)m, 0.0);
  offdiag.assign((size_t)std::max(m - 1, 1), 0.0);
  for (int j = 0; j < m; ++j)
    {
      diag[j] = j == 0 ? 1.0 / alpha[j] : 1.0 / alpha[j] + beta[j - 1] / alpha[j - 1];
      if (j + 1 < m)
        offdiag[j] = std::sqrt(beta[j]) / alpha[j];
    }
}

void pdh_chebyshev_coefficients(int degree, double estimate, double smoothing_range, double *lambda_lo, double *lambda_hi,
                                std::vector<double> &c1, std::vector<double> &c2)
{
  const double hi = 1.2 * estimate, lo = hi / smoothing_range;
  const double theta = (hi + lo) / 2, delta = (hi - lo) / 2, sigma = theta / delta;
  c1.assign((size_t)degree, 0.0);
  c2.assign((size_t)degree, 0.0);
  c2[0] = 1 / theta;
  double rho_old = 1 / sigma;
  for (int k = 1; k < degree; ++k)
    {
      const double rho = 1 / (2 * sigma - rho_old);
      c1[k] = rho * rho_old;
      c2[k] = 2 * rho / delta;
      rho_old = rho;
    }
  *lambda_lo = lo;
  *lambda_hi = hi;
}
```

polydeal_amd/csrc/pdh_plan.h:

```cpp
#pragma once
#include "../../include/polydeal_hip.h"
#include "pdh_dev.h"

#include <algorithm>
#include <cstdint>
#include <cstdlib>
#include <memory>
#include <string>
#include <thread>
#include <vector>

template <class F>
void host_parallel_for(size_t n, F &&fn)
{
  unsigned nt = std::thread::hardware_concurrency();
  if (const char *e = std::getenv("PDH_HOST_THREADS"))
    nt = (unsigned)std::max(1, std::atoi(e));
  nt = std::max(1u, std::min<unsigned>(nt, 64u));
  if (nt == 1 || n < 256)
    {
      for (size_t i = 0; i < n; ++i)
        fn(i);
      return;
    }
  std::vector<std::thread> th;
  const size_t chunk = (n + nt - 1) / nt;
  for (unsigned t = 0; t < nt; ++t)
    {
      const size_t b = (size_t)t * chunk, e = std::min(n, b + chunk);
      if (b >= e)
        break;
      th.emplace_back([&fn, b, e] {
        for (size_t i = b; i < e; ++i)
          fn(i);
      });
    }
  for (auto &t : th)
    t.join();
}

enum class RowKernel { none, rows, terms };

template <class T>
struct UninitAlloc : std::allocator<T>
{
  template <class U>
  struct rebind { using other = UninitAlloc<U>; };
  template <class U, class... A>
  void construct(U *ptr, A &&...a)
  {
    if constexpr (sizeof...(A) == 0)
      ::new ((void *)ptr) U;
    else
      ::new ((void *)ptr) U(std::forward<A>(a)...);
  }
};
using dvec = std::vector<double, UninitAlloc<double>>;

struct Packed
{
  int n = 0, n1d = 0, NT = 0, LB = 0;
  bool tiled = false;
  std::vector<int32_t> midx;
  PdhBasisTab tab;
  std::vector<int32_t> own_agg, own_row, row_len, diag_L, it_own, it_nbr, it_pcnt, it_pos, it_nbr_slot, it_pos_t;
  std::vector<int64_t> row_base, vq_ptr, ap_ptr, it_pbeg;
  std::vector<int64_t> blk_ptr{0};
  std::vector<int32_t> blk_dof;
  int max_row_len = 0;
  dvec vq_x, vq_w;
  std::vector<int64_t> pk_at, pk_fq;
  std::vector<int32_t> pk_cnt, pk_flags;
  std::vector<double> pk_sig;
  int64_t n_ap = 0;
  const double *vqx_h = nullptr, *vqw_h = nullptr;
  int64_t vq_stride_h = 0, n_vq = 0;
  std::vector<int64_t> vq_src, run_ap, run_fq;
  std::vector<int32_t> run_cnt, run_bdry;
  std::vector<int32_t> run_slot, run_nbr, run_blk;
  std::vector<double> run_sig;
  const pdh_cartesian_points *cart = nullptr;
  bool ghost = false;
  const pdh_problem *src = nullptr;
  int64_t nqf_src = 0;
  double ap_x(int d, size_t r, int64_t q) const { return src->fq_x[d * nqf_src + pk_fq[r] + q]; }
  double ap_n(int d, size_t r, int64_t q) const { return ((pk_flags[r] & 1) ? 1.0 : -1.0) * src->fq_n[d * nqf_src + pk_fq[r] + q]; }
  double ap_wself(size_t r, int64_t q) const
  {
    const int64_t i = pk_fq[r] + q;
    if (pk_flags[r] & 2)
      return 2.0 * src->fq_w[i];
    return ((pk_flags[r] & 1) || !src->fq_w_out) ? src->fq_w[i] : src->fq_w_out[i];
  }
  double ap_wcross(size_t r, int64_t q) const
  {
    const int64_t i = pk_fq[r] + q;
    return (pk_flags[r] & 2) ? 0.0 : (src->fq_w_out ? src->fq_w_out[i] : src->fq_w[i]);
  }
  int64_t n_values = 0;
  int n_owned = 0;
  std::vector<int64_t> send_count, recv_count;
  int64_t n_send = 0, n_recv = 0;
  std::vector<int32_t> r21_rlen, r22_slot;
  std::vector<int64_t> r21_src, r21_dst, r22_ptr, r22_src;
};

struct RowsHost
{
  std::vector<int32_t> fr_ptr, fr_pcnt, fr_nbr, fr_axis, fr_blk, fr_flags;
  std::vector<int64_t> fr_pbeg;
  std::vector<double> fr_coord, fr_sigma, fr_nsign;
  std::vector<double> meta;
  int fq_tensor_n = 0;
  bool multi = false;
  int maxe = 16, maxf = 6;
  int maxs = 0;
  bool planar_ok = false;
  std::vector<signed char> fast_j;
};

struct TermsHost
{
  std::vector<double> meta;
  std::vector<int64_t> sf_pt;
  std::vector<int32_t> sf_info, sf_ivl, cell_ivl;
  int maxruns = 0, maxsf = 0, maxsi = 0, maxcell = 0, lds_bytes = 0, split = 0, task_pts = 0;
  int64_t n_cells_in = 0, n_cells_out = 0, n_sf_in = 0, n_sf_out = 0;
};

struct KernelPlan
{
  RowKernel kernel = RowKernel::none;
  RowsHost rows;
  TermsHost terms;
  int vq_n = -1;
  bool tensor_only = false;
  std::string why_rows, why_terms;
};

int pack_problem(std::string &err, const pdh_problem *p, int32_t row_begin, int32_t row_end, Packed &K,
                 int exchange_mode = PDH_EXCHANGE_NONE, const pdh_cartesian_points *cart = nullptr);

struct PlanSwitches
{
  int terms_merge = 1, terms_split = -1;
  bool trace = false, rows_verbose = false, terms_off = false, terms_dgq3_off = false;
  int rows_waves_per_cu = 0, terms_wg_waves = 4;
  size_t rows_lds_pad = 0;
};
PlanSwitches read_plan_switches();

KernelPlan plan_kernels(const pdh_problem *p, const Packed &K, const PlanSwitches &sw);

int combo_group(int dim, int n1d, int nt, int lb);

std::string &pdh_noctx_error();

void pdh_lanczos_tridiagonal(const std::vector<double> &alpha, const std::vector<double> &beta, std::vector<double> &diag,
                             std::vector<double> &offdiag);
void pdh_chebyshev_coefficients(int degree, double estimate, double smoothing_range, double *lambda_lo, double *lambda_hi,
                                std::vector<double> &c1, std::vector<double> &c2);
```

polydeal_amd/csrc/pdh_terms.h:

```cpp
#pragma once
#include "pdh_kernels.h"
#include "pdh_terms_tables.h"

#ifdef PDHT_STAMP
#define PDHT_MARK(k)                                                                                                  \
  do                                                                                                                  \
    {                                                                                                                 \
      const long long tm_ = (long long)__builtin_readcyclecounter();                                                  \
      if (lane == 0 && T.stamps)                                                                                      \
        T.stamps[(int64_t)slot * 16 + (k)] = tm_;                                                                      \
    }                                                                                                                 \
  while (0)
#else
#define PDHT_MARK(k)
#endif

namespace pdht
{
using pdh::static_for;
typedef unsigned int u2_t __attribute__((ext_vector_type(2)));


template <int N1D, int BASIS, int PMAX, bool PAIR = false>
struct TermTasks
{
  static constexpr int TPM = PAIR ? 2 * PMAX : PMAX;
  using K = Kind<N1D, BASIS>;
  static constexpr int NSYM = K::NSYM, SYMS = K::SYMS, FULL = K::FULL, FULLS = K::FULLS;
  const PdhDev &P;
  const double *rec;
  double *Xa, *Da, *Ca;
  double lo0, lo1, lo2, ih0, ih1, ih2;
  int nsfb, fn, tn;
  const double *gr;
  int maxsf, maxcell;
  __device__ __forceinline__ static double sel3(int c, double x0, double x1, double x2) { return c == 0 ? x0 : (c == 1 ? x1 : x2); }
  __device__ __forceinline__ void basis(double t, double *b) const
  {
    static_for<0, N1D>([&](auto k_) {
      constexpr int k = k_;
      double v = P.tab.coef[k][N1D - 1];
      for (int m = N1D - 2; m >= 0; --m)
        v = v * t + P.tab.coef[k][m];
      b[k] = v;
    });
  }
  __device__ __forceinline__ void basis_d(double t, double *b, double *db) const
  {
    static_for<0, N1D>([&](auto k_) {
      constexpr int k = k_;
      double v = P.tab.coef[k][N1D - 1], d = 0.0;
      for (int m = N1D - 2; m >= 0; --m)
        {
          d = d * t + v;
          v = v * t + P.tab.coef[k][m];
        }
      b[k] = v, db[k] = d;
    });
  }
  struct Pts
  {
    double x[PMAX], ws[PMAX], wc[PMAX];
    double ws0, wc0;
    int npts;
  };
  using TPts = Pts;
  using CPts = Pts;
  __device__ __forceinline__ static double pair_sum(double v)
  {
    const int lo = __builtin_amdgcn_mov_dpp(__double2loint(v), 0xB1 , 0xf, 0xf, true);
    const int hi = __builtin_amdgcn_mov_dpp(__double2hiint(v), 0xB1, 0xf, 0xf, true);
    return v + __hiloint2double(hi, lo);
  }
  __device__ __forceinline__ TPts tang_load(int info, int sf, int dir, int half = 0) const
  {
    TPts r;
    const double *g = gr + (2 * sf + dir) * (3 * TPM);
    const int npts = ((info >> (dir ? 15 : 12)) & 7) * fn;
    r.npts = PAIR ? (npts - PMAX * half < 0 ? 0 : (npts - PMAX * half > PMAX ? PMAX : npts - PMAX * half)) : npts;
    r.ws0 = g[TPM];
    r.wc0 = g[2 * TPM];
    const double *gh = g + (PAIR ? PMAX * half : 0);
    static_for<0, PMAX>([&](auto i_) {
      constexpr int al = i_;
      r.x[al] = gh[al];
      r.ws[al] = gh[TPM + al];
      r.wc[al] = gh[2 * TPM + al];
    });
    return r;
  }
  __device__ __forceinline__ double zeta_load(int sf) const { return gr[(2 * maxsf + 3 * maxcell) * (3 * TPM) + sf]; }
  template <bool WANT_D = true, bool WANT_X = true>
  __device__ __forceinline__ void tang_compute(const TPts &r, int sf, int dir, int info, int half = 0) const
  {
    const int run = info & 0xff, c = (info >> 8) & 3;
    const int ti = c == 0 ? 1 : 0, tj = c == 2 ? 1 : 2, ax = dir ? tj : ti;
    const double *re = rec + TERMS_HDR + run * TERMS_ENT;
    const bool interior = (int)__double_as_longlong(re[1]) >= 0;
    const double lo_d = sel3(ax, lo0, lo1, lo2), ih_d = sel3(ax, ih0, ih1, ih2);
    const double loq = re[3 + ax], ihq = re[6 + ax];
    const double sS = dir ? 1.0 / r.ws0 : 1.0, sC = (dir && interior) ? 1.0 / r.wc0 : 1.0;
    double Dm[NSYM], Xm[FULL];
    for (int i = 0; i < NSYM; ++i)
      Dm[i] = 0.0;
    for (int i = 0; i < FULL; ++i)
      Xm[i] = 0.0;
    static_for<0, PMAX>([&](auto i_) {
      constexpr int al = i_;
      if (al < r.npts)
        {
          double bp[N1D], bq[N1D];
          basis((r.x[al] - lo_d) * ih_d - 0.5, bp);
          basis((r.x[al] - loq) * ihq - 0.5, bq);
          const double wS = r.ws[al] * sS, wC = r.wc[al] * sC;
          static_for<0, N1D>([&](auto k_) {
            constexpr int k = k_;
            const double ws = wS * bp[k], wc = wC * bp[k];
            if constexpr (WANT_D)
              static_for<k, N1D>([&](auto l_) { Dm[K::sym(k, l_)] += ws * bp[l_]; });
            if constexpr (WANT_X)
              static_for<0, N1D>([&](auto l_) { Xm[l_ * N1D + k] += wc * bq[l_]; });
          });
        }
    });
    if constexpr (PAIR)
      {
        if constexpr (WANT_D)
          for (int i = 0; i < NSYM; ++i)
            Dm[i] = pair_sum(Dm[i]);
        if constexpr (WANT_X)
          for (int i = 0; i < FULL; ++i)
            Xm[i] = pair_sum(Xm[i]);
        if (half != 0)
          return;
      }
    if constexpr (WANT_D)
      {
        double *dd = Da + (sf * 3 + ax) * SYMS;
        for (int i = 0; i < NSYM; ++i)
          dd[i] = Dm[i];
      }
    if (WANT_X && interior)
      {
        double *xd = Xa + ((sf - nsfb) * 3 + ax) * FULLS;
        for (int i = 0; i < FULL; ++i)
          xd[i] = Xm[i];
      }
  }
  template <bool WANT_D = true, bool WANT_X = true>
  __device__ __forceinline__ void norm_compute(double zeta, int sf, int info) const
  {
    const int run = info & 0xff, c = (info >> 8) & 3;
    const double sg = ((info >> 10) & 1) ? 1.0 : -1.0;
    const double *re = rec + TERMS_HDR + run * TERMS_ENT;
    const bool interior = (int)__double_as_longlong(re[1]) >= 0;
    const double sig = re[2];
    const double lo_c = sel3(c, lo0, lo1, lo2), ih_c = sel3(c, ih0, ih1, ih2);
    const double loq = re[3 + c], ihq = re[6 + c];
    double bp[N1D], dp[N1D], bq[N1D], dq[N1D];
    basis_d((zeta - lo_c) * ih_c - 0.5, bp, dp);
    basis_d((zeta - loq) * ihq - 0.5, bq, dq);
    double *dd = Da + (sf * 3 + c) * SYMS;
    double *xd = Xa + ((sf - nsfb) * 3 + c) * FULLS;
    const double hs = 0.5 * sg * ih_c, hq = 0.5 * sg * ihq;
    static_for<0, N1D>([&](auto k_) {
      constexpr int k = k_;
      if constexpr (WANT_D)
        static_for<k, N1D>([&](auto l_) {
          constexpr int l = l_;
          dd[K::sym(k, l)] = sig * bp[k] * bp[l] - hs * (dp[k] * bp[l] + bp[k] * dp[l]);
        });
      if (WANT_X && interior)
        static_for<0, N1D>([&](auto l_) {
          constexpr int l = l_;
          xd[l * N1D + k] = (hs * dp[k] - sig * bp[k]) * bq[l] - hq * bp[k] * dq[l];
        });
    });
  }
  __device__ __forceinline__ CPts cell_load(int ct, int half = 0) const
  {
    CPts r;
    const double *g = gr + (2 * maxsf + ct) * (3 * TPM);
    r.npts = 0;
    r.ws0 = g[TPM];
    r.wc0 = 0.0;
    const double *gh = g + (PAIR ? PMAX * half : 0);
    static_for<0, PMAX>([&](auto i_) {
      constexpr int i = i_;
      r.x[i] = gh[i];
      r.ws[i] = gh[TPM + i];
      r.wc[i] = 0.0;
      r.npts += r.ws[i] != 0.0 ? 1 : 0;
    });
    return r;
  }
  __device__ __forceinline__ void cell_compute(const CPts &r, int ct, int half = 0) const
  {
    const int cell = ct / 3, d = ct - 3 * cell;
    const double lo_d = sel3(d, lo0, lo1, lo2), ih_d = sel3(d, ih0, ih1, ih2);
    const double sc = d == 0 ? 1.0 : 1.0 / r.ws0;
    double Mm[NSYM], Km[NSYM];
    for (int i = 0; i < NSYM; ++i)
      Mm[i] = Km[i] = 0.0;
    static_for<0, PMAX>([&](auto i_) {
      constexpr int i = i_;
      if (i < r.npts)
        {
          double bp[N1D], dp[N1D];
          basis_d((r.x[i] - lo_d) * ih_d - 0.5, bp, dp);
          const double w = r.ws[i] * sc;
          static_for<0, N1D>([&](auto k_) {
            constexpr int k = k_;
            const double wb = w * bp[k], wd = w * (dp[k] * ih_d);
            static_for<k, N1D>([&](auto l_) {
              Mm[K::sym(k, l_)] += wb * bp[l_];
              Km[K::sym(k, l_)] += wd * (dp[l_] * ih_d);
            });
          });
        }
    });
    if constexpr (PAIR)
      {
        for (int i = 0; i < NSYM; ++i)
          Mm[i] = pair_sum(Mm[i]), Km[i] = pair_sum(Km[i]);
        if (half != 0)
          return;
      }
    if (d == 0 && P.reaction_c != 0.0)
      for (int i = 0; i < NSYM; ++i)
        Km[i] += P.reaction_c * Mm[i];
    double *cd = Ca + (cell * 3 + d) * 2 * SYMS;
    for (int i = 0; i < NSYM; ++i)
      {
        cd[i] = Mm[i];
        cd[SYMS + i] = Km[i];
      }
  }
};

__device__ __forceinline__ void terms_gather_record(const PdhDev &P, const PdhTerms &T, int slot, int tid, int nt, double *__restrict__ out)
{
  const int REC = TERMS_HDR + T.maxruns * TERMS_ENT;
  const double *g = T.meta + (int64_t)slot * REC;
  const int ncell = (int)((__double_as_longlong(g[0]) >> 16) & 0xffff), nsf = (int)__double_as_longlong(g[11]);
  const int64_t vq_b = __double_as_longlong(g[10]);
  const int fn = T.fq_tensor_n, tn = T.vq_tensor_n, pm = T.tpm;
  const int ntt = 2 * nsf, ntc = 3 * ncell;
  const int64_t sfb = (int64_t)slot * T.maxsf;
  for (int it = tid; it < (ntt + ntc) * pm; it += nt)
    {
      const int task = it / pm, al = it - task * pm;
      double x = 0.0, ws = 0.0, wc = 0.0;
      int at;
      if (task < ntt)
        {
          const int sf = task >> 1, dir = task & 1;
          const int info = T.sf_info[sfb + sf];
          const int64_t pb = T.sf_pt[sfb + sf];
          const int c = (info >> 8) & 3;
          const bool fast_j = ((info >> 11) & 1) != 0;
          const int ti = c == 0 ? 1 : 0, tj = c == 2 ? 1 : 2, ax = dir ? tj : ti;
          const int64_t stp = ((dir == 1) == fast_j) ? 1 : fn;
          const int npts = ((info >> (dir ? 15 : 12)) & 7) * fn;
          if (al < npts)
            {
              const int ii = (al >= fn ? 1 : 0) + (al >= 2 * fn ? 1 : 0) + (al >= 3 * fn ? 1 : 0);
              const int64_t q = pb + T.sf_ivl[((sfb + sf) * 2 + dir) * TERMS_MI + ii] + (al - ii * fn) * stp;
              x = P.ap_x[(int64_t)ax * P.ap_stride + q];
              ws = P.ap_wself[q];
              wc = P.ap_wcross[q];
            }
          at = task;
        }
      else
        {
          const int ct = task - ntt, cell = ct / 3, d = ct - 3 * cell;
          const int ii = (al >= tn ? 1 : 0) + (al >= 2 * tn ? 1 : 0) + (al >= 3 * tn ? 1 : 0);
          const int ci = ii < TERMS_MI ? T.cell_ivl[((int64_t)slot * T.maxcell * 3 + ct) * TERMS_MI + ii] : -1;
          if (ci >= 0)
            {
              const int64_t step = d == 0 ? 1 : (d == 1 ? tn : tn * tn);
              const int64_t q = vq_b + (int64_t)ci * (tn * tn * tn) + (al - ii * tn) * step;
              x = P.vq_x[(int64_t)d * P.vq_stride + q];
              ws = P.vq_w[q];
            }
          at = 2 * T.maxsf + ct;
        }
      double *pt = out + at * (3 * pm);
      pt[al] = x;
      pt[pm + al] = ws;
      pt[2 * pm + al] = wc;
    }
  double *zt = out + (2 * T.maxsf + 3 * T.maxcell) * (3 * pm);
  for (int sf = tid; sf < nsf; sf += nt)
    {
      const int info = T.sf_info[sfb + sf];
      zt[sf] = P.ap_x[(int64_t)((info >> 8) & 3) * P.ap_stride + T.sf_pt[sfb + sf]];
      zt[T.maxsf + sf] = __longlong_as_double((long long)info);
    }
}

constexpr int TERMS_WAVES = 3;

template <int N1D, int BASIS, bool SHIFTED, int PMAX, bool SPLIT>
__global__ void __launch_bounds__(PDH_WAVE, TERMS_WAVES) k_terms(const PdhDev P, const PdhTerms T, const int n_owned)
{
  using K = Kind<N1D, BASIS>;
  constexpr int NF = K::NF, NS = K::NS, NSYM = K::NSYM, SYMS = K::SYMS, FULL = K::FULL, FULLS = K::FULLS, NSUB = K::NSUB;
  extern __shared__ __attribute__((aligned(16))) double lds[];
  const int lane = threadIdx.x;
  const int slot = blockIdx.x;
  if (slot >= n_owned)
    return;
  PDHT_MARK(0);
  const int REC = TERMS_HDR + T.maxruns * TERMS_ENT;
  double *rec = lds;
  int *dig = reinterpret_cast<int *>(lds + terms_rec_doubles(T.maxruns));
  double *Xa = lds + terms_rec_doubles(T.maxruns) + ((NF + 1) / 2 + ((NF + 1) / 2 & 1));
  double *Da = SPLIT ? Xa : Xa + (T.maxsi * 3 * FULLS + ((T.maxsi * 3 * FULLS) & 1));
  if constexpr (SPLIT)
    Xa = Da + NF * NF;
  auto sel3 = [](int c, double x0, double x1, double x2) { return c == 0 ? x0 : (c == 1 ? x1 : x2); };
  const double *g = T.meta + (int64_t)slot * REC;
  const long long h0 = __double_as_longlong(g[0]);
  const int ncell = (int)((h0 >> 16) & 0xffff), nsfb = (int)(h0 >> 32);
  const int nsf = (int)__double_as_longlong(g[11]);
  const double lo0 = g[1], lo1 = g[2], lo2 = g[3];
  const double ih0 = g[4], ih1 = g[5], ih2 = g[6];
  const int64_t rbase = __double_as_longlong(g[7]);
  const int rlen = (int)__double_as_longlong(g[8]);
  const int L = (int)__double_as_longlong(g[9]);
  const int fn = T.fq_tensor_n, tn = T.vq_tensor_n;
  const double *gr = T.tdata + (int64_t)slot * T.tstride;
  const double *gr_info = gr + (2 * T.maxsf + 3 * T.maxcell) * (3 * PMAX) + T.maxsf;
  auto desc = [&](int sf, int &info) {
    info = (int)__double_as_longlong(gr_info[sf < T.maxsf ? sf : 0]);
  };
  int infoT = 0, infoN = 0;
  desc(lane, infoN);
  for (int k0 = 0; k0 < T.maxruns * TERMS_ENT; k0 += 4 * PDH_WAVE)
    {
      double rv[4];
      static_for<0, 4>([&](auto i_) {
        const int k = k0 + lane + PDH_WAVE * i_;
        rv[i_] = k < T.maxruns * TERMS_ENT ? g[TERMS_HDR + k] : 0.0;
      });
      static_for<0, 4>([&](auto i_) {
        const int k = k0 + lane + PDH_WAVE * i_;
        if (k < T.maxruns * TERMS_ENT)
          rec[TERMS_HDR + k] = rv[i_];
      });
    }
  if (lane < NF)
    {
      int k0 = 0, k1 = 0, k2 = 0, cnt = 0;
      for (int iz = 0; iz < N1D; ++iz)
        for (int iy = 0; iy < (BASIS == 0 ? N1D : N1D - iz); ++iy)
          for (int ix = 0; ix < (BASIS == 0 ? N1D : N1D - iy - iz); ++ix)
            {
              if (cnt == lane)
                k0 = ix, k1 = iy, k2 = iz;
              ++cnt;
            }
      dig[lane] = k0 | (k1 << 4) | (k2 << 8);
    }
  double *Ca = Da + nsf * 3 * SYMS;
  constexpr bool PAIR = PMAX > 4;
  constexpr int PL = PAIR ? PMAX / 2 : PMAX, TS = PAIR ? 2 : 1;
  using TT = TermTasks<N1D, BASIS, PL, PAIR>;
  using TPts = typename TT::TPts;
  using CPts = typename TT::CPts;
  const TT tt{P, rec, Xa, Da, Ca, lo0, lo1, lo2, ih0, ih1, ih2, nsfb, fn, tn, gr, T.maxsf, T.maxcell};
  const int n1 = 2 * nsf * TS, ncs = PAIR ? (nsf + 1) & ~1 : nsf, n2 = ncs + 3 * ncell * TS;
  auto dec1 = [&](int tid, int &sf, int &dir, int &half) {
    const int task = tid / TS;
    half = tid - task * TS, sf = task >> 1, dir = task & 1;
  };
  auto dec2 = [&](int tid, int &ct, int &half) {
    const int u = tid - ncs;
    ct = u / TS, half = u - ct * TS;
  };
  auto tang_load = [&](int info, int sf, int dir, int half) { return tt.tang_load(info, sf < T.maxsf ? sf : 0, dir, half); };
  auto tang_compute = [&](const TPts &r, int sf, int dir, int info, int half) { tt.template tang_compute<true, !SPLIT>(r, sf, dir, info, half); };
  auto norm_compute = [&](double zeta, int sf, int info) { tt.template norm_compute<true, !SPLIT>(zeta, sf, info); };
  PDHT_MARK(1);
  TPts tp0;
  double zeta0 = 0.0;
  tp0.npts = 0;
  int sfT, dirT, halfT;
  dec1(lane, sfT, dirT, halfT);
  desc(sfT, infoT);
  tp0 = tang_load(infoT, sfT, dirT, halfT);
  CPts cp0;
  for (int i = 0; i < PL; ++i)
    cp0.x[i] = cp0.ws[i] = cp0.wc[i] = 0.0;
  cp0.npts = 0, cp0.ws0 = 1.0, cp0.wc0 = 0.0;
  int ct0 = 0, halfC = 0;
  if (lane < nsf)
    zeta0 = tt.zeta_load(lane);
  else if (lane >= ncs && lane < n2)
    {
      dec2(lane, ct0, halfC);
      cp0 = tt.cell_load(ct0, halfC);
    }
  __builtin_amdgcn_sched_barrier(0);
  PDH_WAVE_SYNC();
  if (lane < n1)
    tang_compute(tp0, sfT, dirT, infoT, halfT);
  for (int t0 = PDH_WAVE; t0 < n1; t0 += PDH_WAVE)
    {
      const int tid = t0 + lane;
      if (tid < n1)
        {
          int info, sf, dir, half;
          dec1(tid, sf, dir, half);
          desc(sf, info);
          const TPts tp = tang_load(info, sf, dir, half);
          tang_compute(tp, sf, dir, info, half);
        }
    }
  PDHT_MARK(2);
  if (lane < nsf)
    norm_compute(zeta0, lane, infoN);
  else if (lane >= ncs && lane < n2)
    tt.cell_compute(cp0, ct0, halfC);
  for (int t0 = PDH_WAVE; t0 < n2; t0 += PDH_WAVE)
    {
      const int tid = t0 + lane;
      if (tid < nsf)
        {
          int info;
          desc(tid, info);
          norm_compute(tt.zeta_load(tid), tid, info);
        }
      else if (tid >= ncs && tid < n2)
        {
          int ct, half;
          dec2(tid, ct, half);
          const CPts cp = tt.cell_load(ct, half);
          tt.cell_compute(cp, ct, half);
        }
    }
  PDH_WAVE_SYNC();
  PDHT_MARK(3);

  {
    double acc[NF];
    for (int r = 0; r < NF; ++r)
      acc[r] = 0.0;
    const int s = lane / NF, j = lane - s * NF;
    const bool on = s < NSUB;
    const int dj = dig[j];
    const int l0 = dj & 15, l1 = (dj >> 4) & 15, l2 = dj >> 8;
    int o0[N1D], o1[N1D], o2[N1D];
    for (int k = 0; k < N1D; ++k)
      {
        o0[k] = K::sym(k, l0);
        o1[k] = K::sym(k, l1) + SYMS;
        o2[k] = K::sym(k, l2) + 2 * SYMS;
      }
    for (int u = on ? s : ncell; u < ncell; u += NSUB)
      {
        const double *b = Ca + u * 6 * SYMS;
        double M0[N1D], K0[N1D], M1[N1D], K1[N1D], M2[N1D], K2[N1D];
        for (int k = 0; k < N1D; ++k)
          {
            M0[k] = b[o0[k]], K0[k] = b[o0[k] + SYMS];
            M1[k] = b[o1[k] + SYMS], K1[k] = b[o1[k] + 2 * SYMS];
            M2[k] = b[o2[k] + 2 * SYMS], K2[k] = b[o2[k] + 3 * SYMS];
          }
        double mm[NS], km[NS];
        static_for<0, N1D>([&](auto k2_) {
          static_for<0, N1D>([&](auto k1_) {
            constexpr int k1 = k1_, k2 = k2_;
            if constexpr (K::pair_ok(k1, k2))
              {
                mm[K::pair(k1, k2)] = M1[k1] * M2[k2];
                km[K::pair(k1, k2)] = K1[k1] * M2[k2] + M1[k1] * K2[k2];
              }
          });
        });
        static_for<0, NF>([&](auto r_) {
          constexpr typename K::Dig g = K::dig(r_);
          acc[r_] += K0[g.k0] * mm[K::pair(g.k1, g.k2)] + M0[g.k0] * km[K::pair(g.k1, g.k2)];
        });
      }
    for (int u = on ? s : nsf; u < nsf; u += NSUB)
      {
        const double *b = Da + u * 3 * SYMS;
        double f0[N1D], f1[N1D], f2[N1D];
        for (int k = 0; k < N1D; ++k)
          f0[k] = b[o0[k]], f1[k] = b[o1[k]], f2[k] = b[o2[k]];
        double yz[NS];
        static_for<0, N1D>([&](auto k2_) {
          static_for<0, N1D>([&](auto k1_) {
            constexpr int k1 = k1_, k2 = k2_;
            if constexpr (K::pair_ok(k1, k2))
// ... 133 lines not shown
```

polydeal_amd/csrc/pdh_terms.hip:

```cpp
#include "pdh_terms.h"
#include "pdh_terms_wg.h"
#include "pdh_launch.h"

using pdht::for_kind;

__global__ void __launch_bounds__(PDH_WAVE) k_terms_gather(const PdhDev P, const PdhTerms T, double *__restrict__ out, const int n_owned)
{
  const int slot = blockIdx.x;
  if (slot < n_owned)
    pdht::terms_gather_record(P, T, slot, threadIdx.x, PDH_WAVE, out + (int64_t)slot * T.tstride);
}
extern "C" hipError_t pdh_launch_terms_gather(const PdhDev *P, const PdhTerms *T, double *out, int count, hipStream_t stream)
{
  if (count <= 0)
    return hipSuccess;
  hipLaunchKernelGGL(k_terms_gather, dim3((unsigned)count), dim3(PDH_WAVE), 0, stream, *P, *T, out, count);
  return hipGetLastError();
}

extern "C" PdhLaunch pdh_resolve_terms(const PdhDev *P, const PdhTerms *T, int count, int wg_waves)
{
  PdhLaunch L{};
  const int basis = P->n == P->n1d * P->n1d * P->n1d ? 0 : 1;
  const bool shifted = P->diag_first != 0, small = T->task_pts <= 4;
  if (P->n1d == 4 && basis == 0)
    pdh_for_bools(
      [&](auto eight_, auto shifted_, auto small_) {
        constexpr int W = decltype(eight_)::value ? 8 : 4, PM = decltype(small_)::value ? 4 : 8;
        const PdhTermsKernel k = pdht::k_terms_wg<W, decltype(shifted_)::value, PM>;
        L = pdh_record(k, count, PDH_WAVE * W, (size_t)T->lds_bytes);
      },
      wg_waves == 8, shifted, small);
  else
    for_kind(P->n1d, basis, [&](auto n_, auto b_) {
      constexpr int N = decltype(n_)::value, B = decltype(b_)::value;
      if (P->n != pdht::Kind<N, B>::NF)
        return;
      pdh_for_bools(
        [&](auto shifted_, auto small_, auto split_) {
          constexpr int PM = decltype(small_)::value ? 4 : 8;
          const PdhTermsKernel k = pdht::k_terms<N, B, decltype(shifted_)::value, PM, decltype(split_)::value>;
          L = pdh_record(k, count, PDH_WAVE, (size_t)T->lds_bytes);
        },
        shifted, small, T->split != 0);
    });
  return L;
}
extern "C" hipError_t pdh_launch_terms(const PdhLaunch *L, const PdhDev *P, const PdhTerms *T, int count, hipStream_t stream)
{
  return pdh_launch_as(PdhTermsKernel(), *L, stream, *P, *T, count);
}
```

polydeal_amd/csrc/pdh_terms_tables.h:

```cpp
#pragma once
#include <stdint.h>
#include <type_traits>

#include "pdh_dev.h"
#define TERMS_MI 4
struct PdhTerms
{
  const double *meta;
  const int64_t *sf_pt;
  const int32_t *sf_info;
  const int32_t *sf_ivl;
  const int32_t *cell_ivl;
  int32_t task_pts;
  const double *tdata;
  int32_t tstride, tpm;
  int32_t maxruns;
  int32_t maxsf, maxsi, maxcell;
  int32_t vq_tensor_n, fq_tensor_n;
  int32_t lds_bytes;
  int32_t split;
  long long *stamps;
};

namespace pdht
{
constexpr int TERMS_HDR = 12, TERMS_ENT = 10;

template <int N1D, int BASIS>
struct Kind
{
  static constexpr int NF = BASIS == 0 ? N1D * N1D * N1D : N1D * (N1D + 1) * (N1D + 2) / 6;
  static constexpr int NS = BASIS == 0 ? N1D * N1D : N1D * (N1D + 1) / 2;
  static constexpr int NSYM = N1D * (N1D + 1) / 2, FULL = N1D * N1D;
  static constexpr int SYMS = NSYM | 1, FULLS = FULL | 1;
  static constexpr int NSUB = 64 / NF > 0 ? 64 / NF : 1;
  struct Dig
  {
    int k0, k1, k2;
  };
  PDH_HD static constexpr Dig dig(int R)
  {
    if (BASIS == 0)
      return Dig{R % N1D, (R / N1D) % N1D, R / (N1D * N1D)};
    int cnt = 0;
    for (int iz = 0; iz < N1D; ++iz)
      for (int iy = 0; iy < N1D - iz; ++iy)
        for (int ix = 0; ix < N1D - iy - iz; ++ix)
          {
            if (cnt == R)
              return Dig{ix, iy, iz};
            ++cnt;
          }
    return Dig{0, 0, 0};
  }
  PDH_HD static constexpr int pair(int k1, int k2) { return BASIS == 0 ? k1 + N1D * k2 : k2 * N1D - k2 * (k2 - 1) / 2 + k1; }
  PDH_HD static constexpr bool pair_ok(int k1, int k2) { return BASIS == 0 || k1 + k2 < N1D; }
  PDH_HD static constexpr int sym(int k, int l) { return k <= l ? l * (l + 1) / 2 + k : k * (k + 1) / 2 + l; }
};

PDH_HD constexpr int terms_rec_doubles(int maxruns) { return (TERMS_HDR + maxruns * TERMS_ENT + 1) & ~1; }
template <int N1D, int BASIS, bool BLOCK_IN_LDS = true, bool SPLIT = false>
PDH_HD constexpr int terms_lds_doubles(int maxruns, int maxsf, int maxsi, int maxcell)
{
  using K = Kind<N1D, BASIS>;
  const int dg = (K::NF + 1) / 2 + ((K::NF + 1) / 2 & 1);
  const int xa = maxsi * 3 * K::FULLS + ((maxsi * 3 * K::FULLS) & 1);
  int da = maxsf * 3 * K::SYMS + maxcell * 6 * K::SYMS;
  if (BLOCK_IN_LDS && SPLIT)
    {
      const int xb = K::NF * K::NF + xa;
      da = da > xb ? da : xb;
      return terms_rec_doubles(maxruns) + dg + da + (da & 1);
    }
  if (BLOCK_IN_LDS)
    da = da > K::NF * K::NF ? da : K::NF * K::NF;
  return terms_rec_doubles(maxruns) + dg + xa + da + (da & 1);
}

PDH_HD constexpr int terms_task_doubles(int maxsf, int maxcell, int pmax)
{
  return (2 * maxsf + 3 * maxcell) * pmax * 3 + 2 * maxsf;
}

PDH_HD constexpr int matfree_off_d(int n1d, int maxsi) { return maxsi * 3 * ((n1d * n1d) | 1); }
PDH_HD constexpr int matfree_off_c(int n1d, int maxsf, int maxsi)
{
  return matfree_off_d(n1d, maxsi) + maxsf * 3 * ((n1d * (n1d + 1) / 2) | 1);
}
PDH_HD constexpr int matfree_rec_doubles(int n1d, int maxsf, int maxsi, int maxcell)
{
  return matfree_off_c(n1d, maxsf, maxsi) + maxcell * 6 * ((n1d * (n1d + 1) / 2) | 1);
}

template <class F>
bool for_kind(int n1d, int basis, F &&f)
{
  using std::integral_constant;
  if (n1d == 4 && basis == 1)
    f(integral_constant<int, 4>{}, integral_constant<int, 1>{});
  else if (n1d == 3 && basis == 0)
    f(integral_constant<int, 3>{}, integral_constant<int, 0>{});
  else if (n1d == 3 && basis == 1)
    f(integral_constant<int, 3>{}, integral_constant<int, 1>{});
  else if (n1d == 2 && basis == 0)
    f(integral_constant<int, 2>{}, integral_constant<int, 0>{});
  else if (n1d == 2 && basis == 1)
    f(integral_constant<int, 2>{}, integral_constant<int, 1>{});
  else
    return false;
  return true;
}

inline int terms_has_kind(int n1d, int basis)
{
  if (n1d == 4 && basis == 0)
    return 2;
  return for_kind(n1d, basis, [](auto, auto) {}) ? 1 : 0;
}

inline int terms_lds_bytes(int n1d, int basis, int maxruns, int maxsf, int maxsi, int maxcell, int split)
{
  int bytes = 0;
  if (n1d == 4 && basis == 0)
    return 8 * terms_lds_doubles<4, 0, false>(maxruns, maxsf, maxsi, maxcell);
  for_kind(n1d, basis, [&](auto n_, auto b_) {
    constexpr int N = decltype(n_)::value, B = decltype(b_)::value;
    bytes = 8 * (split ? terms_lds_doubles<N, B, true, true>(maxruns, maxsf, maxsi, maxcell)
                       : terms_lds_doubles<N, B, true, false>(maxruns, maxsf, maxsi, maxcell));
  });
  return bytes;
}
}
```

polydeal_amd/csrc/pdh_terms_wg.h:

```cpp
#pragma once
#include "pdh_terms.h"

#ifdef PDHT_STAMP
#define PDHW_MARK(k)                                                                                                  \
  do                                                                                                                  \
    {                                                                                                                 \
      const long long tm_ = (long long)__builtin_readcyclecounter();                                                  \
      if (W == 4 && lane == 0 && T.stamps)                                                                            \
        T.stamps[(int64_t)slot * 16 + 4 * wave + (k)] = tm_;                                                           \
    }                                                                                                                 \
  while (0)
#else
#define PDHW_MARK(k)
#endif

namespace pdht
{
constexpr int WG_STORE_AUX = 2;

template <int W, bool SHIFTED, int PMAX>
__global__ void __launch_bounds__(PDH_WAVE *W, 3) k_terms_wg(const PdhDev P, const PdhTerms T, const int n_owned)
{
  constexpr int N1D = 4, BASIS = 0;
  using K = Kind<N1D, BASIS>;
  constexpr int NF = K::NF, SYMS = K::SYMS, FULLS = K::FULLS;
  constexpr int RPW = 64 / W, NK1 = RPW / 4;
  static_assert(NF == 64 && (W == 4 || W == 8), "FE_DGQ(3), four or eight waves per polytope");
  extern __shared__ __attribute__((aligned(16))) double lds[];
  const int lane = threadIdx.x & (PDH_WAVE - 1);
  const int wave = __builtin_amdgcn_readfirstlane(threadIdx.x >> 6);
  const int slot = blockIdx.x;
  if (slot >= n_owned)
    return;
  PDHW_MARK(0);
  const int REC = TERMS_HDR + T.maxruns * TERMS_ENT;
  double *rec = lds;
  double *Xa = lds + terms_rec_doubles(T.maxruns) + ((NF + 1) / 2 + ((NF + 1) / 2 & 1));
  double *Da = Xa + (T.maxsi * 3 * FULLS + ((T.maxsi * 3 * FULLS) & 1));
  const double *g = T.meta + (int64_t)slot * REC;
  const long long h0 = __double_as_longlong(g[0]);
  const int ncell = (int)((h0 >> 16) & 0xffff), nsfb = (int)(h0 >> 32);
  const int nsf = (int)__double_as_longlong(g[11]);
  const double lo0 = g[1], lo1 = g[2], lo2 = g[3];
  const double ih0 = g[4], ih1 = g[5], ih2 = g[6];
  const int64_t rbase = __double_as_longlong(g[7]);
  const int rlen = (int)__double_as_longlong(g[8]);
  const int L = (int)__double_as_longlong(g[9]);
  const int fn = T.fq_tensor_n, tn = T.vq_tensor_n;
  const double *gr = T.tdata + (int64_t)slot * T.tstride;
  const double *gr_info = gr + (2 * T.maxsf + 3 * T.maxcell) * (3 * PMAX) + T.maxsf;
  for (int k = threadIdx.x; k < T.maxruns * TERMS_ENT; k += PDH_WAVE * W)
    rec[TERMS_HDR + k] = g[TERMS_HDR + k];
  double *Ca = Da + nsf * 3 * SYMS;
  constexpr bool PAIR = PMAX > 4;
  constexpr int PL = PAIR ? PMAX / 2 : PMAX, TS = PAIR ? 2 : 1;
  using TT = TermTasks<N1D, BASIS, PL, PAIR>;
  const TT tt{P, rec, Xa, Da, Ca, lo0, lo1, lo2, ih0, ih1, ih2, nsfb, fn, tn, gr, T.maxsf, T.maxcell};
  auto desc = [&](int sf, int &info) { info = (int)__double_as_longlong(gr_info[sf < T.maxsf ? sf : 0]); };
  {
    constexpr int H = W / 2;
    const bool first_kind = wave < H;
    const int hw = first_kind ? wave : wave - H;
    const int ncs = PAIR ? (nsf + 1) & ~1 : nsf;
    const int ntask = first_kind ? 2 * nsf * TS : ncs + 3 * ncell * TS;
    const int share = ((ntask + H - 1) / H + 1) & ~1;
    const int t_begin = hw * share, t_end = t_begin + share < ntask ? t_begin + share : ntask;
    auto dec1 = [&](int tid, int &sf, int &dir, int &half) {
      const int task = tid / TS;
      half = tid - task * TS, sf = task >> 1, dir = task & 1;
    };
    auto dec2 = [&](int tid, int &ct, int &half) {
      const int u = tid - ncs;
      ct = u / TS, half = u - ct * TS;
    };
    const int tid0 = t_begin + lane;
    const bool on0 = tid0 < t_end;
    int info0 = 0, a0 = 0, b0 = 0, h0_ = 0;
    typename TT::TPts tp0;
    typename TT::CPts cp0;
    double zeta0 = 0.0;
    for (int i = 0; i < PL; ++i)
      tp0.x[i] = tp0.ws[i] = tp0.wc[i] = cp0.x[i] = cp0.ws[i] = cp0.wc[i] = 0.0;
    tp0.npts = cp0.npts = 0;
    tp0.ws0 = tp0.wc0 = cp0.ws0 = 1.0, cp0.wc0 = 0.0;
    if (first_kind)
      {
        dec1(on0 ? tid0 : 0, a0, b0, h0_);
        desc(a0, info0);
        tp0 = tt.tang_load(info0, a0 < T.maxsf ? a0 : 0, b0, h0_);
      }
    else if (on0 && tid0 < nsf)
      {
        desc(tid0, info0);
        zeta0 = tt.zeta_load(tid0);
      }
    else if (on0 && tid0 >= ncs)
      {
        dec2(tid0, a0, h0_);
        cp0 = tt.cell_load(a0, h0_);
      }
    __syncthreads();
    if (first_kind)
      {
        if (on0)
          tt.tang_compute(tp0, a0, b0, info0, h0_);
        for (int tid = tid0 + PDH_WAVE; tid < t_end; tid += PDH_WAVE)
          {
            int info, sf, dir, half;
            dec1(tid, sf, dir, half);
            desc(sf, info);
            const typename TT::TPts tp = tt.tang_load(info, sf, dir, half);
            tt.tang_compute(tp, sf, dir, info, half);
          }
      }
    else
      {
        if (on0 && tid0 < nsf)
          tt.norm_compute(zeta0, tid0, info0);
        else if (on0 && tid0 >= ncs)
          tt.cell_compute(cp0, a0, h0_);
        for (int tid = tid0 + PDH_WAVE; tid < t_end; tid += PDH_WAVE)
          {
            if (tid < nsf)
              {
                int info;
                desc(tid, info);
                tt.norm_compute(tt.zeta_load(tid), tid, info);
              }
            else if (tid >= ncs)
              {
                int ct, half;
                dec2(tid, ct, half);
                const typename TT::CPts cp = tt.cell_load(ct, half);
                tt.cell_compute(cp, ct, half);
              }
          }
      }
  }
  __syncthreads();
  PDHW_MARK(1);

  const int R0 = RPW * wave;
  const int k2 = RPW == 16 ? wave : wave >> 1;
  const int K1B = RPW == 16 ? 0 : 2 * (wave & 1);
  const int m0 = L >> 6, nblk = rlen >> 6;
  const int first_int = nsfb > 0 ? 1 : 0;
  const __amdgpu_buffer_rsrc_t vrs = __builtin_amdgcn_make_buffer_rsrc(P.values + rbase, 0, NF * rlen * 8, 0x00020000);
  auto row_store = [&](double v, uint32_t lane_bytes, uint32_t row_bytes) {
    __builtin_amdgcn_raw_buffer_store_b64(__builtin_bit_cast(u2_t, v), vrs, (int)lane_bytes, (int)row_bytes, WG_STORE_AUX);
  };
  const uint32_t row0_bytes = (uint32_t)R0 * (uint32_t)rlen * 8u, rstep = (uint32_t)rlen * 8u;
  auto add_term = [&](double (&acc)[RPW], const double (&f0)[4], const double (&f1)[NK1], double f2) __attribute__((always_inline)) {
    double yz[NK1];
    static_for<0, NK1>([&](auto i_) { yz[i_] = f1[i_] * f2; });
    static_for<0, RPW>([&](auto r_) {
      constexpr int r = r_;
      acc[r] += f0[r & 3] * yz[r >> 2];
    });
  };
  auto coupling = [&](double (&acc)[RPW], int fl, int col, bool on) __attribute__((always_inline)) {
    const long long e0 = __double_as_longlong(rec[TERMS_HDR + (first_int + fl) * TERMS_ENT]);
    const int ns = on ? (int)(e0 >> 32) : 0;
    const double *xb = Xa + ((int)(uint32_t)e0 - nsfb) * 3 * FULLS;
    const int q0 = (col & 3) * 4, q1 = ((col >> 2) & 3) * 4 + FULLS + K1B, q2 = (col >> 4) * 4 + 2 * FULLS + k2;
    for (int st = 0; __any(st < ns); ++st)
      {
        if (st < ns)
          {
            double f0[4], f1[NK1];
            for (int k = 0; k < 4; ++k)
              f0[k] = xb[q0 + k];
            for (int i = 0; i < NK1; ++i)
              f1[i] = xb[q1 + i];
            add_term(acc, f0, f1, xb[q2]);
          }
        xb += 3 * FULLS;
      }
  };
  double own[RPW];
  static_for<0, RPW>([&](auto r_) { own[r_] = 0.0; });
  {
    const int l0 = lane & 3, l1 = (lane >> 2) & 3, l2 = lane >> 4;
    int o0[4], o1[NK1];
    for (int k = 0; k < 4; ++k)
      o0[k] = K::sym(k, l0);
    for (int i = 0; i < NK1; ++i)
      o1[i] = K::sym(K1B + i, l1) + SYMS;
    const int o2 = K::sym(k2, l2) + 2 * SYMS;
    for (int u = 0; u < ncell; ++u)
      {
        const double *b = Ca + u * 6 * SYMS;
        double M0[4], K0[4], mm[NK1], km[NK1];
        const double M2 = b[o2 + 2 * SYMS], K2 = b[o2 + 3 * SYMS];
        for (int k = 0; k < 4; ++k)
          M0[k] = b[o0[k]], K0[k] = b[o0[k] + SYMS];
        for (int i = 0; i < NK1; ++i)
          {
            const double M1 = b[o1[i] + SYMS], K1 = b[o1[i] + 2 * SYMS];
            mm[i] = M1 * M2;
            km[i] = K1 * M2 + M1 * K2;
          }
        static_for<0, RPW>([&](auto r_) {
          constexpr int r = r_;
          own[r] += K0[r & 3] * mm[r >> 2] + M0[r & 3] * km[r >> 2];
        });
      }
    for (int u = 0; u < nsf; ++u)
      {
        const double *b = Da + u * 3 * SYMS;
        double f0[4], f1[NK1];
        for (int k = 0; k < 4; ++k)
          f0[k] = b[o0[k]];
        for (int i = 0; i < NK1; ++i)
          f1[i] = b[o1[i]];
        add_term(own, f0, f1, b[o2]);
      }
  }
  PDHW_MARK(2);
  if constexpr (!SHIFTED)
    {
      for (int b = 0; b < nblk; ++b)
        {
          double acc[RPW];
          if (b == m0)
            static_for<0, RPW>([&](auto r_) { acc[r_] = own[r_]; });
          else
            {
              static_for<0, RPW>([&](auto r_) { acc[r_] = 0.0; });
              coupling(acc, b < m0 ? b : b - 1, lane, true);
            }
          uint32_t rowrun = row0_bytes + (uint32_t)b * 512u;
          static_for<0, RPW>([&](auto r_) {
            row_store(acc[r_], (uint32_t)lane * 8u, rowrun);
            rowrun += rstep;
          });
        }
    }
  else
    {
      double dg[RPW];
      {
        double left63[RPW];
        static_for<0, RPW>([&](auto r_) { left63[r_] = 0.0; });
        if (m0 > 0)
          coupling(left63, m0 - 1, 63, true);
        uint32_t rowrun = row0_bytes + (uint32_t)m0 * 512u;
        static_for<0, RPW>([&](auto r_) {
          constexpr int r = r_;
          const int R = R0 + r;
          dg[r] = __hiloint2double(__builtin_amdgcn_readlane(__double2hiint(own[r]), R), __builtin_amdgcn_readlane(__double2loint(own[r]), R));
          const bool diag = lane == R;
          double lv = left63[r];
          asm volatile("" : "+v"(lv));
          const double v = (diag && m0 > 0) ? lv : own[r];
          const uint32_t off = diag ? 0u : (lane < R ? (uint32_t)(lane + 1) * 8u : (uint32_t)lane * 8u);
          row_store(v, off, rowrun);
          rowrun += rstep;
        });
      }
      for (int m = 0; m < m0; ++m)
        {
          double acc[RPW];
          static_for<0, RPW>([&](auto r_) { acc[r_] = 0.0; });
          const bool l0_ = lane == 0;
          coupling(acc, l0_ ? (m > 0 ? m - 1 : 0) : m, l0_ ? 63 : lane - 1, !(l0_ && m == 0));
          if (m == 0)
            static_for<0, RPW>([&](auto r_) {
              double dv = dg[r_];
              asm volatile("" : "+v"(dv));
              acc[r_] = l0_ ? dv : acc[r_];
            });
          uint32_t rowrun = row0_bytes + (uint32_t)m * 512u;
          static_for<0, RPW>([&](auto r_) {
            row_store(acc[r_], (uint32_t)lane * 8u, rowrun);
            rowrun += rstep;
          });
        }
      for (int b = m0 + 1; b < nblk; ++b)
        {
          double acc[RPW];
          static_for<0, RPW>([&](auto r_) { acc[r_] = 0.0; });
          coupling(acc, b - 1, lane, true);
          uint32_t rowrun = row0_bytes + (uint32_t)b * 512u;
          static_for<0, RPW>([&](auto r_) {
            row_store(acc[r_], (uint32_t)lane * 8u, rowrun);
            rowrun += rstep;
          });
        }
    }
  PDHW_MARK(3);
}
}
```

Before: 1.514 billion.

## Make FE_DGQ(3) term kernel persistent with builder waves and double-buffered LDS tables

Turns the FE_DGQ(3) term kernel into a persistent kernel. Each compute unit runs one workgroup that holds writer waves plus four extra builder waves, and loops over polytopes using a work counter and a double buffer of LDS tables. Builders stage the next polytope's tables while the writers store rows for the current one, so table preparation overlaps with the global writes. The default grows to eight writer waves, and the launch requests half the compute unit's LDS to force one workgroup per CU. The checksum is also changed to a two-pass reduction without atomics. The risks are lower occupancy, extra synchronisation, and failing setup on devices whose LDS or occupancy queries do not match.

```diff
diff --git a/polydeal_amd/csrc/pdh_capi.cpp b/polydeal_amd/csrc/pdh_capi.cpp
--- a/polydeal_amd/csrc/pdh_capi.cpp
+++ b/polydeal_amd/csrc/pdh_capi.cpp
@@ -406,13 +406,16 @@
   const size_t n_stamps = (size_t)std::max(K.n_owned, 1) * 16;
   PDH_TRY(device_buffer(ctx, n_stamps, &T.stamps, "term kernel: stamps"));
   PDH_HIP(ctx, hipMemset(T.stamps, 0, n_stamps * sizeof(long long)));
+  PDH_TRY(device_buffer(ctx, 16, &T.sched, "term kernel: work counter"));
+  PDH_HIP(ctx, hipMemset(T.sched, 0, 16 * sizeof(unsigned int)));
   ctx->prob.terms_merge[0] = TH.n_cells_in, ctx->prob.terms_merge[1] = TH.n_cells_out;
   ctx->prob.terms_merge[2] = TH.n_sf_in, ctx->prob.terms_merge[3] = TH.n_sf_out;
   return PDH_OK;
 }
 
-static void resolve_launches(pdh_ctx *ctx, const Packed &K, const PlanSwitches &sw, int cus)
-{
+static void resolve_launches(pdh_ctx *ctx, const Packed &K, const PlanSwitches &sw, int cus, const char **why_row)
+{
+  *why_row = nullptr;
   pdh_ctx::Problem &pr = ctx->prob;
   const PdhDev &D = pr.dev;
   const bool reaction = D.reaction_c != 0.0;
@@ -425,7 +428,12 @@
   if (pr.row_kernel == RowKernel::rows)
     pr.row = pdh_resolve_rows(&D, &pr.rows, pr.n_owned, cus, sw.rows_waves_per_cu, sw.rows_lds_pad, sw.rows_verbose, &pr.row_zero_sched);
   else if (pr.row_kernel == RowKernel::terms)
-    pr.row = pdh_resolve_terms(&D, &pr.terms, pr.n_owned, sw.terms_wg_waves);
+    {
+      const char *why = nullptr;
+      pr.row = pdh_resolve_terms(&D, &pr.terms, pr.n_owned, cus, sw.terms_wg_waves, sw.terms_wg_batch, &why);
+      if (!pr.row.kernel)
+        *why_row = why;
+    }
 }
 
 static int set_problem_impl(pdh_ctx *ctx, const pdh_problem *p, int32_t row_begin, int32_t row_end, const pdh_cartesian_points *cart);
@@ -500,7 +508,10 @@
     }
   ctx->prob.row_kernel = plan->kernel;
   ctx->prob.why_terms = plan->why_terms;
-  resolve_launches(ctx, K, sw, cus);
+  const char *why_row = nullptr;
+  resolve_launches(ctx, K, sw, cus, &why_row);
+  if (why_row)
+    return fail(ctx, PDH_EUNSUPPORTED, std::string("the row kernel chosen for this problem cannot be launched on this device: ") + why_row);
   ctx->prob.resident = true;
   ctx->ev_used = 0;
   guard.done = true;
@@ -813,7 +824,7 @@
   if (!out4)
     return fail(ctx, PDH_EINVAL, "out4 is NULL");
   PDH_HIP(ctx, hipSetDevice(ctx->device));
-  double *d = ctx->checksum.get<double>(4);
+  double *d = ctx->checksum.get<double>(pdh_checksum_doubles());
   if (!d)
     return fail(ctx, PDH_EDEVICE, "pdh_values_checksum: out of device memory");
   hipError_t e = pdh_launch_checksum(ctx->prob.dev.values, ctx->prob.n_values, d, ctx->stream);
diff --git a/polydeal_amd/csrc/pdh_exchange.hip b/polydeal_amd/csrc/pdh_exchange.hip
--- a/polydeal_amd/csrc/pdh_exchange.hip
+++ b/polydeal_amd/csrc/pdh_exchange.hip
@@ -47,6 +47,41 @@
   return hipGetLastError();
 }
 
+constexpr int CHECKSUM_BLOCKS = 2048;
+__device__ __forceinline__ void checksum_block_reduce(double s, double sa, double mx, double bad, double *__restrict__ o)
+{
+  __shared__ double part[4][4];
+  for (int d = 32; d > 0; d >>= 1)
+    {
+      s += __shfl_down(s, d);
+      sa += __shfl_down(sa, d);
+      bad += __shfl_down(bad, d);
+      mx = fmax(mx, __shfl_down(mx, d));
+    }
+  const int w = threadIdx.x >> 6;
+  if ((threadIdx.x & 63) == 0)
+    part[w][0] = s, part[w][1] = sa, part[w][2] = mx, part[w][3] = bad;
+  __syncthreads();
+  if (threadIdx.x == 0)
+    {
+      o[0] = (part[0][0] + part[1][0]) + (part[2][0] + part[3][0]);
+      o[1] = (part[0][1] + part[1][1]) + (part[2][1] + part[3][1]);
+      o[2] = fmax(fmax(part[0][2], part[1][2]), fmax(part[2][2], part[3][2]));
+      o[3] = (part[0][3] + part[1][3]) + (part[2][3] + part[3][3]);
+    }
+}
+__global__ void __launch_bounds__(256) k_checksum_final(const double *__restrict__ partials, double *__restrict__ out)
+{
+  double s = 0.0, sa = 0.0, mx = 0.0, bad = 0.0;
+  for (int b = threadIdx.x; b < CHECKSUM_BLOCKS; b += 256)
+    {
+      s += partials[4 * b + 0];
+      sa += partials[4 * b + 1];
+      mx = fmax(mx, partials[4 * b + 2]);
+      bad += partials[4 * b + 3];
+    }
+  checksum_block_reduce(s, sa, mx, bad, out);
+}
 __global__ void __launch_bounds__(256) k_checksum(const double *__restrict__ v, const int64_t n, double *__restrict__ out)
 {
   double s = 0.0, sa = 0.0, mx = 0.0, bad = 0.0;
@@ -62,28 +97,17 @@
       else
         bad += 1.0;
     }
-  for (int o = 32; o > 0; o >>= 1)
-    {
-      s += __shfl_down(s, o);
-      sa += __shfl_down(sa, o);
-      bad += __shfl_down(bad, o);
-      mx = fmax(mx, __shfl_down(mx, o));
-    }
-  if ((threadIdx.x & 63) == 0)
-    {
-      atomicAdd(out + 0, s);
-      atomicAdd(out + 1, sa);
-      atomicAdd(out + 3, bad);
-      atomicMax(reinterpret_cast<unsigned long long *>(out + 2), (unsigned long long)__double_as_longlong(mx));
-    }
+  checksum_block_reduce(s, sa, mx, bad, out + 4 * blockIdx.x);
 }
 
-extern "C" hipError_t pdh_launch_checksum(const double *values, int64_t n, double *d_out4, hipStream_t stream)
+extern "C" size_t pdh_checksum_doubles() { return 4 + 4 * (size_t)CHECKSUM_BLOCKS; }
+extern "C" hipError_t pdh_launch_checksum(const double *values, int64_t n, double *d_out, hipStream_t stream)
 {
-  hipError_t e = hipMemsetAsync(d_out4, 0, 4 * sizeof(double), stream);
+  hipError_t e = hipMemsetAsync(d_out, 0, 4 * sizeof(double), stream);
   if (e != hipSuccess || n <= 0)
     return e;
-  hipLaunchKernelGGL(k_checksum, dim3(2048), dim3(256), 0, stream, values, n, d_out4);
+  hipLaunchKernelGGL(k_checksum, dim3(CHECKSUM_BLOCKS), dim3(256), 0, stream, values, n, d_out + 4);
+  hipLaunchKernelGGL(k_checksum_final, dim3(1), dim3(256), 0, stream, d_out + 4, d_out);
   return hipGetLastError();
 }
 
diff --git a/polydeal_amd/csrc/pdh_launch.h b/polydeal_amd/csrc/pdh_launch.h
--- a/polydeal_amd/csrc/pdh_launch.h
+++ b/polydeal_amd/csrc/pdh_launch.h
@@ -80,7 +80,7 @@
 hipError_t pdh_launch_rows(const PdhLaunch *L, bool zero_sched, const PdhDev *P, const PdhRows *R, const double *mtab, int count,
                            hipStream_t stream);
 
-PdhLaunch pdh_resolve_terms(const PdhDev *P, const PdhTerms *T, int count, int wg_waves);
+PdhLaunch pdh_resolve_terms(const PdhDev *P, const PdhTerms *T, int count, int cus, int wg_waves, int wg_batch, const char **why);
 hipError_t pdh_launch_terms(const PdhLaunch *L, const PdhDev *P, const PdhTerms *T, int count, hipStream_t stream);
 hipError_t pdh_launch_terms_gather(const PdhDev *P, const PdhTerms *T, double *out, int count, hipStream_t stream);
 
@@ -103,7 +103,8 @@
 hipError_t pdh_launch_ghost_apply(const PdhDev *P, const double *recv, int n_r21, const int64_t *r21_src, const int64_t *r21_dst,
                                   const int32_t *r21_rlen, int n_r22, const int64_t *r22_ptr, const int64_t *r22_src,
                                   const int32_t *r22_slot, hipStream_t stream);
-hipError_t pdh_launch_checksum(const double *values, int64_t n, double *d_out4, hipStream_t stream);
+size_t pdh_checksum_doubles();
+hipError_t pdh_launch_checksum(const double *values, int64_t n, double *d_out, hipStream_t stream);
 
 hipError_t pdh_launch_vmult(const PdhSolveArgs *A, const double *x, double *y, double *part, hipStream_t stream);
 hipError_t pdh_launch_block_inverse(const PdhSolveArgs *A, double *dinv, int32_t *flag, hipStream_t stream);
diff --git a/polydeal_amd/csrc/pdh_plan.cpp b/polydeal_amd/csrc/pdh_plan.cpp
--- a/polydeal_amd/csrc/pdh_plan.cpp
+++ b/polydeal_amd/csrc/pdh_plan.cpp
@@ -1417,7 +1417,8 @@
   s.terms_dgq3_off = first("PDH_TERMS_DGQ3") == '0';
   s.rows_waves_per_cu = getenv("PDH_ROWS_WAVES_PER_CU") ? atoi(getenv("PDH_ROWS_WAVES_PER_CU")) : 0;
   s.rows_lds_pad = getenv("PDH_ROWS_LDS_PAD") ? (size_t)atol(getenv("PDH_ROWS_LDS_PAD")) : 0;
-  s.terms_wg_waves = getenv("PDH_TERMS_WG_WAVES") && atoi(getenv("PDH_TERMS_WG_WAVES")) == 8 ? 8 : 4;
+  s.terms_wg_waves = getenv("PDH_TERMS_WG_WAVES") && atoi(getenv("PDH_TERMS_WG_WAVES")) == 4 ? 4 : 8;
+  s.terms_wg_batch = getenv("PDH_TERMS_WG_BATCH") ? atoi(getenv("PDH_TERMS_WG_BATCH")) : 0;
   return s;
 }
 
diff --git a/polydeal_amd/csrc/pdh_plan.h b/polydeal_amd/csrc/pdh_plan.h
--- a/polydeal_amd/csrc/pdh_plan.h
+++ b/polydeal_amd/csrc/pdh_plan.h
@@ -145,7 +145,7 @@
 {
   int terms_merge = 1, terms_split = -1;
   bool trace = false, rows_verbose = false, terms_off = false, terms_dgq3_off = false;
-  int rows_waves_per_cu = 0, terms_wg_waves = 4;
+  int rows_waves_per_cu = 0, terms_wg_waves = 8, terms_wg_batch = 0;
   size_t rows_lds_pad = 0;
 };
 PlanSwitches read_plan_switches();
diff --git a/polydeal_amd/csrc/pdh_terms.h b/polydeal_amd/csrc/pdh_terms.h
--- a/polydeal_amd/csrc/pdh_terms.h
+++ b/polydeal_amd/csrc/pdh_terms.h
@@ -193,6 +193,42 @@
       r.npts += r.ws[i] != 0.0 ? 1 : 0;
     });
     return r;
+  }
+  template <bool CROSS>
+  __device__ __forceinline__ static Pts task_request(const double *g, int half)
+  {
+    Pts r;
+    r.npts = 0;
+    r.ws0 = r.wc0 = 0.0;
+    const double *gh = g + (PAIR ? PMAX * half : 0);
+    static_for<0, PMAX>([&](auto i_) {
+      constexpr int i = i_;
+      r.x[i] = gh[i];
+      r.ws[i] = gh[TPM + i];
+      r.wc[i] = CROSS ? gh[2 * TPM + i] : 0.0;
+    });
+    return r;
+  }
+  __device__ __forceinline__ static void task_first_weights(Pts &r)
+  {
+    auto even = [](double v) {
+      const int lo = __builtin_amdgcn_mov_dpp(__double2loint(v), 0xA0 , 0xf, 0xf, true);
+      const int hi = __builtin_amdgcn_mov_dpp(__double2hiint(v), 0xA0, 0xf, 0xf, true);
+      return __hiloint2double(hi, lo);
+    };
+    r.ws0 = PAIR ? even(r.ws[0]) : r.ws[0];
+    r.wc0 = PAIR ? even(r.wc[0]) : r.wc[0];
+  }
+  __device__ __forceinline__ static int tang_npts(int info, int dir, int fn, int half)
+  {
+    const int npts = ((info >> (dir ? 15 : 12)) & 7) * fn;
+    return PAIR ? (npts - PMAX * half < 0 ? 0 : (npts - PMAX * half > PMAX ? PMAX : npts - PMAX * half)) : npts;
+  }
+  __device__ __forceinline__ static int cell_npts(const Pts &r)
+  {
+    int n = 0;
+    static_for<0, PMAX>([&](auto i_) { n += r.ws[i_] != 0.0 ? 1 : 0; });
+    return n;
   }
   __device__ __forceinline__ void cell_compute(const CPts &r, int ct, int half = 0) const
   {
diff --git a/polydeal_amd/csrc/pdh_terms.hip b/polydeal_amd/csrc/pdh_terms.hip
--- a/polydeal_amd/csrc/pdh_terms.hip
+++ b/polydeal_amd/csrc/pdh_terms.hip
@@ -1,6 +1,8 @@
 #include "pdh_terms.h"
 #include "pdh_terms_wg.h"
 #include "pdh_launch.h"
+
+#include <algorithm>
 
 using pdht::for_kind;
 
@@ -18,19 +20,50 @@
   return hipGetLastError();
 }
 
-extern "C" PdhLaunch pdh_resolve_terms(const PdhDev *P, const PdhTerms *T, int count, int wg_waves)
+extern "C" PdhLaunch pdh_resolve_terms(const PdhDev *P, const PdhTerms *T, int count, int cus, int wg_waves, int wg_batch, const char **why)
 {
   PdhLaunch L{};
+  *why = "no instantiation of the term kernel for this element, or a grid beyond 2^31 - 1 workgroups";
   const int basis = P->n == P->n1d * P->n1d * P->n1d ? 0 : 1;
   const bool shifted = P->diag_first != 0, small = T->task_pts <= 4;
   if (P->n1d == 4 && basis == 0)
     pdh_for_bools(
       [&](auto eight_, auto shifted_, auto small_) {
         constexpr int W = decltype(eight_)::value ? 8 : 4, PM = decltype(small_)::value ? 4 : 8;
+        constexpr unsigned block = PDH_WAVE * (W + pdht::WG_BUILDERS);
         const PdhTermsKernel k = pdht::k_terms_wg<W, decltype(shifted_)::value, PM>;
-        L = pdh_record(k, count, PDH_WAVE * W, (size_t)T->lds_bytes);
+        int dev = 0, cu_lds = 0;
+        if (hipGetDevice(&dev) != hipSuccess ||
+            hipDeviceGetAttribute(&cu_lds, hipDeviceAttributeMaxSharedMemoryPerMultiprocessor, dev) != hipSuccess || cu_lds <= 0)
+          {
+            (void)hipGetLastError();
+            *why = "FE_DGQ(3) term kernel: the device does not report the LDS of a compute unit";
+            return;
+          }
+        const size_t lds = (size_t)cu_lds / 2 + 1024;
+        if (lds < 2 * (size_t)T->lds_bytes + 64)
+          {
+            *why = "FE_DGQ(3) term kernel: two table buffers do not fit the LDS request that keeps a workgroup alone on its compute unit";
+            return;
+          }
+        int per_cu = 0;
+        if (hipFuncSetAttribute((const void *)k, hipFuncAttributeMaxDynamicSharedMemorySize, (int)lds) != hipSuccess)
+          {
+            (void)hipGetLastError();
+            *why = "FE_DGQ(3) term kernel: the device refuses the dynamic LDS of its workgroup (hipFuncSetAttribute)";
+            return;
+          }
+        if (hipOccupancyMaxActiveBlocksPerMultiprocessor(&per_cu, k, (int)block, lds) != hipSuccess || per_cu != 1)
+          {
+            (void)hipGetLastError();
+            *why = "FE_DGQ(3) term kernel: the occupancy query does not answer one workgroup per compute unit";
+            return;
+          }
+        const long long n = count > 0 ? count : 0;
+        const long long grid = wg_batch > 0 ? (n + wg_batch - 1) / wg_batch : std::min<long long>(n, cus > 0 ? cus : 1);
+        L = pdh_record(k, grid, block, lds);
       },
-      wg_waves == 8, shifted, small);
+      wg_waves != 4, shifted, small);
   else
     for_kind(P->n1d, basis, [&](auto n_, auto b_) {
       constexpr int N = decltype(n_)::value, B = decltype(b_)::value;
diff --git a/polydeal_amd/csrc/pdh_terms_tables.h b/polydeal_amd/csrc/pdh_terms_tables.h
--- a/polydeal_amd/csrc/pdh_terms_tables.h
+++ b/polydeal_amd/csrc/pdh_terms_tables.h
@@ -20,6 +20,7 @@
   int32_t lds_bytes;
   int32_t split;
   long long *stamps;
+  unsigned int *sched;
 };
 
 namespace pdht
diff --git a/polydeal_amd/csrc/pdh_terms_wg.h b/polydeal_amd/csrc/pdh_terms_wg.h
--- a/polydeal_amd/csrc/pdh_terms_wg.h
+++ b/polydeal_amd/csrc/pdh_terms_wg.h
@@ -2,154 +2,192 @@
 #include "pdh_terms.h"
 
 #ifdef PDHT_STAMP
-#define PDHW_MARK(k)                                                                                                  \
+#define PDHW_MARK(s, base, k)                                                                                         \
   do                                                                                                                  \
     {                                                                                                                 \
       const long long tm_ = (long long)__builtin_readcyclecounter();                                                  \
-      if (W == 4 && lane == 0 && T.stamps)                                                                            \
-        T.stamps[(int64_t)slot * 16 + 4 * wave + (k)] = tm_;                                                           \
+      if ((base) >= 0 && lane == 0 && T.stamps)                                                                       \
+        T.stamps[(int64_t)(s) * 16 + (base) + (k)] = tm_;                                                              \
     }                                                                                                                 \
   while (0)
 #else
-#define PDHW_MARK(k)
+#define PDHW_MARK(s, base, k)
 #endif
 
 namespace pdht
 {
 constexpr int WG_STORE_AUX = 2;
+constexpr int WG_BUILDERS = 4;
+constexpr int WG_TICKET = 2;
 
 template <int W, bool SHIFTED, int PMAX>
-__global__ void __launch_bounds__(PDH_WAVE *W, 3) k_terms_wg(const PdhDev P, const PdhTerms T, const int n_owned)
+__global__ void __launch_bounds__(PDH_WAVE *(W + WG_BUILDERS), 1) k_terms_wg(const PdhDev P, const PdhTerms T, const int n_owned)
 {
   constexpr int N1D = 4, BASIS = 0;
   using K = Kind<N1D, BASIS>;
   constexpr int NF = K::NF, SYMS = K::SYMS, FULLS = K::FULLS;
   constexpr int RPW = 64 / W, NK1 = RPW / 4;
-  static_assert(NF == 64 && (W == 4 || W == 8), "FE_DGQ(3), four or eight waves per polytope");
+  static_assert(NF == 64 && (W == 4 || W == 8), "FE_DGQ(3), four or eight writer waves");
   extern __shared__ __attribute__((aligned(16))) double lds[];
+  __shared__ int seq[4];
   const int lane = threadIdx.x & (PDH_WAVE - 1);
   const int wave = __builtin_amdgcn_readfirstlane(threadIdx.x >> 6);
-  const int slot = blockIdx.x;
-  if (slot >= n_owned)
-    return;
-  PDHW_MARK(0);
-  const int REC = TERMS_HDR + T.maxruns * TERMS_ENT;
-  double *rec = lds;
-  double *Xa = lds + terms_rec_doubles(T.maxruns) + ((NF + 1) / 2 + ((NF + 1) / 2 & 1));
-  double *Da = Xa + (T.maxsi * 3 * FULLS + ((T.maxsi * 3 * FULLS) & 1));
-  const double *g = T.meta + (int64_t)slot * REC;
-  const long long h0 = __double_as_longlong(g[0]);
-  const int ncell = (int)((h0 >> 16) & 0xffff), nsfb = (int)(h0 >> 32);
-  const int nsf = (int)__double_as_longlong(g[11]);
-  const double lo0 = g[1], lo1 = g[2], lo2 = g[3];
-  const double ih0 = g[4], ih1 = g[5], ih2 = g[6];
-  const int64_t rbase = __double_as_longlong(g[7]);
-  const int rlen = (int)__double_as_longlong(g[8]);
-  const int L = (int)__double_as_longlong(g[9]);
-  const int fn = T.fq_tensor_n, tn = T.vq_tensor_n;
-  const double *gr = T.tdata + (int64_t)slot * T.tstride;
-  const double *gr_info = gr + (2 * T.maxsf + 3 * T.maxcell) * (3 * PMAX) + T.maxsf;
-  for (int k = threadIdx.x; k < T.maxruns * TERMS_ENT; k += PDH_WAVE * W)
-    rec[TERMS_HDR + k] = g[TERMS_HDR + k];
-  double *Ca = Da + nsf * 3 * SYMS;
+  const int s0 = blockIdx.x, s1 = s0 + (int)gridDim.x;
+  const int NENT = T.maxruns * TERMS_ENT, REC = TERMS_HDR + NENT;
+  const int stride = T.lds_bytes >> 3;
+  const int XA_OFF = terms_rec_doubles(T.maxruns) + ((NF + 1) / 2 + ((NF + 1) / 2 & 1));
+  const int DA_OFF = XA_OFF + (T.maxsi * 3 * FULLS + ((T.maxsi * 3 * FULLS) & 1));
+  auto hdr = [](double hv, int i) {
+    return __hiloint2double(__builtin_amdgcn_readlane(__double2hiint(hv), i), __builtin_amdgcn_readlane(__double2loint(hv), i));
+  };
   constexpr bool PAIR = PMAX > 4;
   constexpr int PL = PAIR ? PMAX / 2 : PMAX, TS = PAIR ? 2 : 1;
   using TT = TermTasks<N1D, BASIS, PL, PAIR>;
-  const TT tt{P, rec, Xa, Da, Ca, lo0, lo1, lo2, ih0, ih1, ih2, nsfb, fn, tn, gr, T.maxsf, T.maxcell};
-  auto desc = [&](int sf, int &info) { info = (int)__double_as_longlong(gr_info[sf < T.maxsf ? sf : 0]); };
-  {
-    constexpr int H = W / 2;
-    const bool first_kind = wave < H;
-    const int hw = first_kind ? wave : wave - H;
-    const int ncs = PAIR ? (nsf + 1) & ~1 : nsf;
-    const int ntask = first_kind ? 2 * nsf * TS : ncs + 3 * ncell * TS;
-    const int share = ((ntask + H - 1) / H + 1) & ~1;
-    const int t_begin = hw * share, t_end = t_begin + share < ntask ? t_begin + share : ntask;
-    auto dec1 = [&](int tid, int &sf, int &dir, int &half) {
-      const int task = tid / TS;
-      half = tid - task * TS, sf = task >> 1, dir = task & 1;
-    };
-    auto dec2 = [&](int tid, int &ct, int &half) {
-      const int u = tid - ncs;
-      ct = u / TS, half = u - ct * TS;
-    };
-    const int tid0 = t_begin + lane;
-    const bool on0 = tid0 < t_end;
-    int info0 = 0, a0 = 0, b0 = 0, h0_ = 0;
-    typename TT::TPts tp0;
-    typename TT::CPts cp0;
-    double zeta0 = 0.0;
-    for (int i = 0; i < PL; ++i)
-      tp0.x[i] = tp0.ws[i] = tp0.wc[i] = cp0.x[i] = cp0.ws[i] = cp0.wc[i] = 0.0;
-    tp0.npts = cp0.npts = 0;
-    tp0.ws0 = tp0.wc0 = cp0.ws0 = 1.0, cp0.wc0 = 0.0;
-    if (first_kind)
+
+  if (wave >= W)
+    {
+      const int bw = wave - W;
+      __builtin_amdgcn_s_setprio(3);
+#ifdef PDHT_STAMP
+      const int sbase = bw == 0 ? 6 : (bw == WG_BUILDERS - 1 ? 9 : -1);
+#endif
+      const int tid0 = (bw < 2 ? bw * PDH_WAVE : 0) + lane;
+      const int task0 = tid0 / TS, half0 = tid0 - task0 * TS;
+      const int sf0 = bw < 2 ? task0 >> 1 : tid0, dir0 = task0 & 1;
+      const int sf0c = sf0 < T.maxsf ? sf0 : 0, ct0c = task0 < 3 * T.maxcell ? task0 : 0;
+      const int info_off = (2 * T.maxsf + 3 * T.maxcell) * (3 * PMAX) + T.maxsf;
+      constexpr int NC = 2;
+      struct Req
       {
-        dec1(on0 ? tid0 : 0, a0, b0, h0_);
-        desc(a0, info0);
-        tp0 = tt.tang_load(info0, a0 < T.maxsf ? a0 : 0, b0, h0_);
-      }
-    else if (on0 && tid0 < nsf)
-      {
-        desc(tid0, info0);
-        zeta0 = tt.zeta_load(tid0);
-      }
-    else if (on0 && tid0 >= ncs)
-      {
-        dec2(tid0, a0, h0_);
-        cp0 = tt.cell_load(a0, h0_);
-      }
-    __syncthreads();
-    if (first_kind)
-      {
-        if (on0)
-          tt.tang_compute(tp0, a0, b0, info0, h0_);
-        for (int tid = tid0 + PDH_WAVE; tid < t_end; tid += PDH_WAVE)
-          {
-            int info, sf, dir, half;
-            dec1(tid, sf, dir, half);
-            desc(sf, info);
-            const typename TT::TPts tp = tt.tang_load(info, sf, dir, half);
-            tt.tang_compute(tp, sf, dir, info, half);
-          }
-      }
-    else
-      {
-        if (on0 && tid0 < nsf)
-          tt.norm_compute(zeta0, tid0, info0);
-        else if (on0 && tid0 >= ncs)
-          tt.cell_compute(cp0, a0, h0_);
-        for (int tid = tid0 + PDH_WAVE; tid < t_end; tid += PDH_WAVE)
-          {
-            if (tid < nsf)
-              {
-                int info;
-                desc(tid, info);
-                tt.norm_compute(tt.zeta_load(tid), tid, info);
-              }
-            else if (tid >= ncs)
-              {
-                int ct, half;
-                dec2(tid, ct, half);
+        typename TT::Pts p;
+        int info;
+        double c[NC];
+      };
+      auto request = [&](int s) __attribute__((always_inline)) {
+        Req r;
+        const int sc = s < n_owned ? s : n_owned - 1;
+        const double *g = T.meta + (int64_t)sc * REC;
+        const double *gr = T.tdata + (int64_t)sc * T.tstride;
+        static_for<0, NC>([&](auto i_) {
+          const int k = lane + PDH_WAVE * i_;
+          r.c[i_] = 0.0;
+          if (PDH_WAVE * i_ < REC)
+            r.c[i_] = g[k < REC ? k : 0];
+        });
+        r.info = reinterpret_cast<const int *>(gr + info_off + sf0c)[0];
+        if (bw < 2)
+          r.p = TT::template task_request<true>(gr + (2 * sf0c + dir0) * (3 * PMAX), half0);
+        else if (bw == 3)
+          r.p = TT::template task_request<false>(gr + (2 * T.maxsf + ct0c) * (3 * PMAX), half0);
+        else
+          {
+            r.p = typename TT::Pts{};
+            r.p.x[0] = gr[(2 * T.maxsf + 3 * T.maxcell) * (3 * PMAX) + sf0c];
+          }
+        return r;
+      };
+      auto build = [&](const Req &r, int s, double *buf) __attribute__((always_inline)) {
+        double *rec = buf, *Xa = buf + XA_OFF, *Da = buf + DA_OFF;
+        const double hv = r.c[0];
+        const long long h0 = __double_as_longlong(hdr(hv, 0));
+        const int ncell = (int)((h0 >> 16) & 0xffff), nsfb = (int)(h0 >> 32);
+        const int nsf = (int)__double_as_longlong(hdr(hv, 11));
+        const double lo0 = hdr(hv, 1), lo1 = hdr(hv, 2), lo2 = hdr(hv, 3);
+        const double ih0 = hdr(hv, 4), ih1 = hdr(hv, 5), ih2 = hdr(hv, 6);
+        const int fn = T.fq_tensor_n, tn = T.vq_tensor_n;
+        const double *g = T.meta + (int64_t)s * REC;
+        const double *gr = T.tdata + (int64_t)s * T.tstride;
+        double *Ca = Da + nsf * 3 * SYMS;
+        static_for<0, NC>([&](auto i_) {
+          const int k = lane + PDH_WAVE * i_;
+          if (k < REC)
+            rec[k] = r.c[i_];
+        });
+        for (int k = NC * PDH_WAVE + lane; k < REC; k += PDH_WAVE)
+          rec[k] = g[k];
+        PDH_WAVE_SYNC();
+        const TT tt{P, rec, Xa, Da, Ca, lo0, lo1, lo2, ih0, ih1, ih2, nsfb, fn, tn, gr, T.maxsf, T.maxcell};
+        auto desc = [&](int sf) { return (int)__double_as_longlong(gr[info_off + (sf < T.maxsf ? sf : 0)]); };
+        const int info0 = r.info;
+        typename TT::Pts p = r.p;
+        TT::task_first_weights(p);
+        if (bw < 2)
+          {
+            const int n1 = 2 * nsf * TS;
+            if (tid0 < n1)
+              {
+                p.npts = TT::tang_npts(info0, dir0, fn, half0);
+                tt.tang_compute(p, sf0, dir0, info0, half0);
+              }
+            for (int tid = tid0 + 2 * PDH_WAVE; tid < n1; tid += 2 * PDH_WAVE)
+              {
+                const int task = tid / TS, half = tid - task * TS, sf = task >> 1, dir = task & 1;
+                const int info = desc(sf);
+                const typename TT::TPts tp = tt.tang_load(info, sf, dir, half);
+                tt.tang_compute(tp, sf, dir, info, half);
+              }
+          }
+        else if (bw == 2)
+          {
+            if (tid0 < nsf)
+              tt.norm_compute(r.p.x[0], tid0, info0);
+            for (int tid = tid0 + PDH_WAVE; tid < nsf; tid += PDH_WAVE)
+              tt.norm_compute(tt.zeta_load(tid), tid, desc(tid));
+          }
+        else
+          {
+            const int n3 = 3 * ncell * TS;
+            if (tid0 < n3)
+              {
+                p.npts = TT::cell_npts(p);
+                tt.cell_compute(p, task0, half0);
+              }
+            for (int tid = tid0 + PDH_WAVE; tid < n3; tid += PDH_WAVE)
+              {
+                const int ct = tid / TS, half = tid - ct * TS;
                 const typename TT::CPts cp = tt.cell_load(ct, half);
                 tt.cell_compute(cp, ct, half);
               }
           }
-      }
-  }
-  __syncthreads();
-  PDHW_MARK(1);
-
+      };
+      int s_cur = s0, s_nxt = s1;
+      Req rq = request(s_cur);
+      for (int j = 0;; ++j)
+        {
+          const bool fetch = bw == WG_TICKET && s_nxt < n_owned;
+          unsigned tick = 0;
+          if (fetch && lane == 0)
+            tick = __hip_atomic_fetch_add(T.sched, 1u, __ATOMIC_RELAXED, __HIP_MEMORY_SCOPE_AGENT);
+          const Req rn = request(s_nxt);
+          PDHW_MARK(s_cur < n_owned ? s_cur : 0, s_cur < n_owned ? sbase : -1, 0);
+          if (s_cur < n_owned)
+            build(rq, s_cur, lds + (j & 1) * stride);
+          if (bw == WG_TICKET && lane == 0)
+            seq[(j + 2) & 3] = fetch ? 2 * (int)gridDim.x + (int)tick : n_owned;
+          PDHW_MARK(s_cur < n_owned ? s_cur : 0, s_cur < n_owned ? sbase : -1, 1);
+          __syncthreads();
+          PDHW_MARK(s_cur < n_owned ? s_cur : 0, s_cur < n_owned ? sbase : -1, 2);
+          if (s_cur >= n_owned)
+            break;
+          s_cur = s_nxt;
+          rq = rn;
+          s_nxt = __builtin_amdgcn_readfirstlane(seq[(j + 2) & 3]);
+        }
+      if (bw == WG_TICKET && lane == 0)
+        if (__hip_atomic_fetch_add(T.sched + 1, 1u, __ATOMIC_ACQ_REL, __HIP_MEMORY_SCOPE_AGENT) == gridDim.x - 1)
+          {
+            __hip_atomic_store(T.sched, 0u, __ATOMIC_RELAXED, __HIP_MEMORY_SCOPE_AGENT);
+            __hip_atomic_store(T.sched + 1, 0u, __ATOMIC_RELEASE, __HIP_MEMORY_SCOPE_AGENT);
+          }
+      return;
+    }
+
+#ifdef PDHT_STAMP
+  const int sbase = wave == 0 ? 0 : (wave == W - 1 ? 3 : -1);
+#endif
   const int R0 = RPW * wave;
   const int k2 = RPW == 16 ? wave : wave >> 1;
   const int K1B = RPW == 16 ? 0 : 2 * (wave & 1);
-  const int m0 = L >> 6, nblk = rlen >> 6;
-  const int first_int = nsfb > 0 ? 1 : 0;
-  const __amdgpu_buffer_rsrc_t vrs = __builtin_amdgcn_make_buffer_rsrc(P.values + rbase, 0, NF * rlen * 8, 0x00020000);
-  auto row_store = [&](double v, uint32_t lane_bytes, uint32_t row_bytes) {
-    __builtin_amdgcn_raw_buffer_store_b64(__builtin_bit_cast(u2_t, v), vrs, (int)lane_bytes, (int)row_bytes, WG_STORE_AUX);
-  };
-  const uint32_t row0_bytes = (uint32_t)R0 * (uint32_t)rlen * 8u, rstep = (uint32_t)rlen * 8u;
   auto add_term = [&](double (&acc)[RPW], const double (&f0)[4], const double (&f1)[NK1], double f2) __attribute__((always_inline)) {
     double yz[NK1];
     static_for<0, NK1>([&](auto i_) { yz[i_] = f1[i_] * f2; });
@@ -158,136 +196,163 @@
       acc[r] += f0[r & 3] * yz[r >> 2];
     });
   };
-  auto coupling = [&](double (&acc)[RPW], int fl, int col, bool on) __attribute__((always_inline)) {
-    const long long e0 = __double_as_longlong(rec[TERMS_HDR + (first_int + fl) * TERMS_ENT]);
-    const int ns = on ? (int)(e0 >> 32) : 0;
-    const double *xb = Xa + ((int)(uint32_t)e0 - nsfb) * 3 * FULLS;
-    const int q0 = (col & 3) * 4, q1 = ((col >> 2) & 3) * 4 + FULLS + K1B, q2 = (col >> 4) * 4 + 2 * FULLS + k2;
-    for (int st = 0; __any(st < ns); ++st)
+  int s = s0;
+  __syncthreads();
+  for (int step = 0;; ++step)
+    {
+      if (step > 0)
+        s = step == 1 ? s1 : __builtin_amdgcn_readfirstlane(seq[step & 3]);
+      if (s >= n_owned)
+        break;
+      PDHW_MARK(s, sbase, 0);
+      const double *rec = lds + (step & 1) * stride, *Xa = rec + XA_OFF, *Da = rec + DA_OFF;
+      const double hv = rec[lane < TERMS_HDR ? lane : 0];
+      const long long h0 = __double_as_longlong(hdr(hv, 0));
+      const int ncell = (int)((h0 >> 16) & 0xffff), nsfb = (int)(h0 >> 32);
+      const int nsf = (int)__double_as_longlong(hdr(hv, 11));
+      const int64_t rbase = __double_as_longlong(hdr(hv, 7));
+      const int rlen = (int)__double_as_longlong(hdr(hv, 8));
+      const int L = (int)__double_as_longlong(hdr(hv, 9));
+      const double *Ca = Da + nsf * 3 * SYMS;
+      const int m0 = L >> 6, nblk = rlen >> 6;
+      const int first_int = nsfb > 0 ? 1 : 0;
+      const __amdgpu_buffer_rsrc_t vrs = __builtin_amdgcn_make_buffer_rsrc(P.values + rbase, 0, NF * rlen * 8, 0x00020000);
+      auto row_store = [&](double v, uint32_t lane_bytes, uint32_t row_bytes) {
+        __builtin_amdgcn_raw_buffer_store_b64(__builtin_bit_cast(u2_t, v), vrs, (int)lane_bytes, (int)row_bytes, WG_STORE_AUX);
+      };
+      const uint32_t row0_bytes = (uint32_t)R0 * (uint32_t)rlen * 8u, rstep = (uint32_t)rlen * 8u;
+      auto coupling = [&](double (&acc)[RPW], int fl, int col, bool on) __attribute__((always_inline)) {
+        const long long e0 = __double_as_longlong(rec[TERMS_HDR + (first_int + fl) * TERMS_ENT]);
+        const int ns = on ? (int)(e0 >> 32) : 0;
+        const double *xb = Xa + ((int)(uint32_t)e0 - nsfb) * 3 * FULLS;
+        const int q0 = (col & 3) * 4, q1 = ((col >> 2) & 3) * 4 + FULLS + K1B, q2 = (col >> 4) * 4 + 2 * FULLS + k2;
+        for (int st = 0; __any(st < ns); ++st)
+          {
+            if (st < ns)
+              {
+                double f0[4], f1[NK1];
+                for (int k = 0; k < 4; ++k)
+                  f0[k] = xb[q0 + k];
+                for (int i = 0; i < NK1; ++i)
+                  f1[i] = xb[q1 + i];
+                add_term(acc, f0, f1, xb[q2]);
+              }
+            xb += 3 * FULLS;
+          }
+      };
+      double own[RPW];
+      static_for<0, RPW>([&](auto r_) { own[r_] = 0.0; });
       {
-        if (st < ns)
-          {
+        const int l0 = lane & 3, l1 = (lane >> 2) & 3, l2 = lane >> 4;
+        int o0[4], o1[NK1];
+        for (int k = 0; k < 4; ++k)
+          o0[k] = K::sym(k, l0);
+        for (int i = 0; i < NK1; ++i)
+          o1[i] = K::sym(K1B + i, l1) + SYMS;
+        const int o2 = K::sym(k2, l2) + 2 * SYMS;
+        for (int u = 0; u < ncell; ++u)
+          {
+            const double *b = Ca + u * 6 * SYMS;
+            double M0[4], K0[4], mm[NK1], km[NK1];
+            const double M2 = b[o2 + 2 * SYMS], K2 = b[o2 + 3 * SYMS];
+            for (int k = 0; k < 4; ++k)
+              M0[k] = b[o0[k]], K0[k] = b[o0[k] + SYMS];
+            for (int i = 0; i < NK1; ++i)
+              {
+                const double M1 = b[o1[i] + SYMS], K1 = b[o1[i] + 2 * SYMS];
+                mm[i] = M1 * M2;
+                km[i] = K1 * M2 + M1 * K2;
+              }
+            static_for<0, RPW>([&](auto r_) {
+              constexpr int r = r_;
+              own[r] += K0[r & 3] * mm[r >> 2] + M0[r & 3] * km[r >> 2];
+            });
+          }
+        for (int u = 0; u < nsf; ++u)
+          {
+            const double *b = Da + u * 3 * SYMS;
             double f0[4], f1[NK1];
             for (int k = 0; k < 4; ++k)
-              f0[k] = xb[q0 + k];
+              f0[k] = b[o0[k]];
             for (int i = 0; i < NK1; ++i)
-              f1[i] = xb[q1 + i];
-            add_term(acc, f0, f1, xb[q2]);
-          }
-        xb += 3 * FULLS;
+              f1[i] = b[o1[i]];
+            add_term(own, f0, f1, b[o2]);
+          }
       }
-  };
-  double own[RPW];
-  static_for<0, RPW>([&](auto r_) { own[r_] = 0.0; });
-  {
-    const int l0 = lane & 3, l1 = (lane >> 2) & 3, l2 = lane >> 4;
-    int o0[4], o1[NK1];
-    for (int k = 0; k < 4; ++k)
-      o0[k] = K::sym(k, l0);
-    for (int i = 0; i < NK1; ++i)
-      o1[i] = K::sym(K1B + i, l1) + SYMS;
-    const int o2 = K::sym(k2, l2) + 2 * SYMS;
-    for (int u = 0; u < ncell; ++u)
-      {
-        const double *b = Ca + u * 6 * SYMS;
-        double M0[4], K0[4], mm[NK1], km[NK1];
-        const double M2 = b[o2 + 2 * SYMS], K2 = b[o2 + 3 * SYMS];
-        for (int k = 0; k < 4; ++k)
-          M0[k] = b[o0[k]], K0[k] = b[o0[k] + SYMS];
-        for (int i = 0; i < NK1; ++i)
-          {
-            const double M1 = b[o1[i] + SYMS], K1 = b[o1[i] + 2 * SYMS];
-            mm[i] = M1 * M2;
-            km[i] = K1 * M2 + M1 * K2;
-          }
-        static_for<0, RPW>([&](auto r_) {
-          constexpr int r = r_;
-          own[r] += K0[r & 3] * mm[r >> 2] + M0[r & 3] * km[r >> 2];
-        });
-      }
-    for (int u = 0; u < nsf; ++u)
-      {
-        const double *b = Da + u * 3 * SYMS;
-        double f0[4], f1[NK1];
-        for (int k = 0; k < 4; ++k)
-          f0[k] = b[o0[k]];
-        for (int i = 0; i < NK1; ++i)
-          f1[i] = b[o1[i]];
-        add_term(own, f0, f1, b[o2]);
-      }
-  }
-  PDHW_MARK(2);
-  if constexpr (!SHIFTED)
-    {
-      for (int b = 0; b < nblk; ++b)
+      if constexpr (!SHIFTED)
         {
-          double acc[RPW];
-          if (b == m0)
-            static_for<0, RPW>([&](auto r_) { acc[r_] = own[r_]; });
-          else
+          for (int b = 0; b < nblk; ++b)
             {
+              double acc[RPW];
+              if (b == m0)
+                static_for<0, RPW>([&](auto r_) { acc[r_] = own[r_]; });
+              else
+                {
+                  static_for<0, RPW>([&](auto r_) { acc[r_] = 0.0; });
+                  coupling(acc, b < m0 ? b : b - 1, lane, true);
+                }
+              uint32_t rowrun = row0_bytes + (uint32_t)b * 512u;
+              static_for<0, RPW>([&](auto r_) {
+                row_store(acc[r_], (uint32_t)lane * 8u, rowrun);
+                rowrun += rstep;
+              });
+            }
+        }
+      else
+        {
+          double dg[RPW];
+          {
+            double left63[RPW];
+            static_for<0, RPW>([&](auto r_) { left63[r_] = 0.0; });
+            if (m0 > 0)
+              coupling(left63, m0 - 1, 63, true);
+            uint32_t rowrun = row0_bytes + (uint32_t)m0 * 512u;
+            static_for<0, RPW>([&](auto r_) {
+              constexpr int r = r_;
+              const int R = R0 + r;
+              dg[r] = __hiloint2double(__builtin_amdgcn_readlane(__double2hiint(own[r]), R), __builtin_amdgcn_readlane(__double2loint(own[r]), R));
+              const bool diag = lane == R;
+              double lv = left63[r];
+              asm volatile("" : "+v"(lv));
+              const double v = (diag && m0 > 0) ? lv : own[r];
+              const uint32_t off = diag ? 0u : (lane < R ? (uint32_t)(lane + 1) * 8u : (uint32_t)lane * 8u);
+              row_store(v, off, rowrun);
+              rowrun += rstep;
+            });
+          }
+          for (int m = 0; m < m0; ++m)
+            {
+              double acc[RPW];
               static_for<0, RPW>([&](auto r_) { acc[r_] = 0.0; });
-              coupling(acc, b < m0 ? b : b - 1, lane, true);
+              const bool l0_ = lane == 0;
+              coupling(acc, l0_ ? (m > 0 ? m - 1 : 0) : m, l0_ ? 63 : lane - 1, !(l0_ && m == 0));
+              if (m == 0)
+                static_for<0, RPW>([&](auto r_) {
+                  double dv = dg[r_];
+                  asm volatile("" : "+v"(dv));
+                  acc[r_] = l0_ ? dv : acc[r_];
+                });
+              uint32_t rowrun = row0_bytes + (uint32_t)m * 512u;
+              static_for<0, RPW>([&](auto r_) {
+                row_store(acc[r_], (uint32_t)lane * 8u, rowrun);
+                rowrun += rstep;
+              });
             }
-          uint32_t rowrun = row0_bytes + (uint32_t)b * 512u;
-          static_for<0, RPW>([&](auto r_) {
-            row_store(acc[r_], (uint32_t)lane * 8u, rowrun);
-            rowrun += rstep;
-          });
+          for (int b = m0 + 1; b < nblk; ++b)
+            {
+              double acc[RPW];
+              static_for<0, RPW>([&](auto r_) { acc[r_] = 0.0; });
+              coupling(acc, b - 1, lane, true);
+              uint32_t rowrun = row0_bytes + (uint32_t)b * 512u;
+              static_for<0, RPW>([&](auto r_) {
+                row_store(acc[r_], (uint32_t)lane * 8u, rowrun);
+                rowrun += rstep;
+              });
+            }
         }
+      PDHW_MARK(s, sbase, 1);
+      __syncthreads();
+      PDHW_MARK(s, sbase, 2);
     }
-  else
-    {
-      double dg[RPW];
-      {
-        double left63[RPW];
-        static_for<0, RPW>([&](auto r_) { left63[r_] = 0.0; });
-        if (m0 > 0)
-          coupling(left63, m0 - 1, 63, true);
-        uint32_t rowrun = row0_bytes + (uint32_t)m0 * 512u;
-        static_for<0, RPW>([&](auto r_) {
-          constexpr int r = r_;
-          const int R = R0 + r;
-          dg[r] = __hiloint2double(__builtin_amdgcn_readlane(__double2hiint(own[r]), R), __builtin_amdgcn_readlane(__double2loint(own[r]), R));
-          const bool diag = lane == R;
-          double lv = left63[r];
-          asm volatile("" : "+v"(lv));
-          const double v = (diag && m0 > 0) ? lv : own[r];
-          const uint32_t off = diag ? 0u : (lane < R ? (uint32_t)(lane + 1) * 8u : (uint32_t)lane * 8u);
-          row_store(v, off, rowrun);
-          rowrun += rstep;
-        });
-      }
-      for (int m = 0; m < m0; ++m)
-        {
-          double acc[RPW];
-          static_for<0, RPW>([&](auto r_) { acc[r_] = 0.0; });
-          const bool l0_ = lane == 0;
-          coupling(acc, l0_ ? (m > 0 ? m - 1 : 0) : m, l0_ ? 63 : lane - 1, !(l0_ && m == 0));
-          if (m == 0)
-            static_for<0, RPW>([&](auto r_) {
-              double dv = dg[r_];
-              asm volatile("" : "+v"(dv));
-              acc[r_] = l0_ ? dv : acc[r_];
-            });
-          uint32_t rowrun = row0_bytes + (uint32_t)m * 512u;
-          static_for<0, RPW>([&](auto r_) {
-            row_store(acc[r_], (uint32_t)lane * 8u, rowrun);
-            rowrun += rstep;
-          });
-        }
-      for (int b = m0 + 1; b < nblk; ++b)
-        {
-          double acc[RPW];
-          static_for<0, RPW>([&](auto r_) { acc[r_] = 0.0; });
-          coupling(acc, b - 1, lane, true);
-          uint32_t rowrun = row0_bytes + (uint32_t)b * 512u;
-          static_for<0, RPW>([&](auto r_) {
-            row_store(acc[r_], (uint32_t)lane * 8u, rowrun);
-            rowrun += rstep;
-          });
-        }
-    }
-  PDHW_MARK(3);
 }
 }
```

Result: faster. 1.810 billion, median of 6 (+19.5%).
